# zerr0o/whisper-burn

Measured on AMD Instinct MI355X. Metric: real-time factor (audio-s/wall-s) Whisper Large-V3 Q4 @1/2/4/8 MI355X, higher is better.
Workload: dtype fp16x2

## Files before the change

### include/whisper_amd.h

```cpp
#ifndef WHISPER_AMD_H
#define WHISPER_AMD_H

#include <stddef.h>
#include <stdint.h>

#include "wq4.h"

#ifdef __cplusplus
extern "C" {
#endif

typedef struct wa_model wa_model;

typedef enum wa_variant { WA_LARGE_V3 = 0, WA_MEDIUM = 1, WA_TINY_TEST = 2 } wa_variant;

enum {
  WA_CFG_N_MELS = 0,
  WA_CFG_N_AUDIO_CTX,
  WA_CFG_N_AUDIO_STATE,
  WA_CFG_N_AUDIO_HEAD,
  WA_CFG_N_AUDIO_LAYER,
  WA_CFG_N_TEXT_CTX,
  WA_CFG_N_TEXT_STATE,
  WA_CFG_N_TEXT_HEAD,
  WA_CFG_N_TEXT_LAYER,
  WA_CFG_N_VOCAB,
  WA_CFG_N_LANG,
  WA_CFG_COUNT
};

const char* wa_last_error(void);

wq4_status wa_model_create_synthetic(int device, int variant, uint64_t seed, int max_batch, wq4_precision prec,
                                     wa_model** out);
wq4_status wa_model_create_synthetic_ex(int device, int variant, uint64_t seed, int max_batch, wq4_precision prec,
                                        int weight_type, wa_model** out);
int wa_model_weight_type(const wa_model* m);
int wa_model_wide_range(const wa_model* m);
wq4_status wa_model_create_from_gguf(int device, const char* path, int variant, int max_batch, wq4_precision prec,
                                     wa_model** out);
void wa_model_destroy(wa_model* m);

typedef struct wa_gguf wa_gguf;
wq4_status wa_gguf_open(const char* path, wa_gguf** out);
void wa_gguf_close(wa_gguf* g);
int wa_gguf_version(const wa_gguf* g);
int64_t wa_gguf_tensor_count(const wa_gguf* g);
wq4_status wa_gguf_tensor_info(const wa_gguf* g, int64_t index, char* name, size_t name_cap, int* ndims,
                               uint64_t* dims, int* type, uint64_t* offset, uint64_t* nbytes);
wq4_status wa_gguf_tensor_data(const wa_gguf* g, const char* name, uint8_t* out, size_t cap);
wq4_status wa_model_config(const wa_model* m, int32_t* cfg );
size_t wa_model_device_bytes(const wa_model* m);

wq4_status wa_transcribe(wa_model* m, const float* mel_dev, int n_clips, int lang_token, int max_tokens,
                         int eot_stop, int32_t* tokens_out, int32_t* n_tokens_out, void* stream);

wq4_status wa_transcribe_batches(wa_model* m, const float* mel_dev, int n_batches, int n_clips, int lang_token,
                                 int max_tokens, int eot_stop, int32_t* tokens_out, int32_t* n_tokens_out,
                                 void* stream);
wq4_status wa_last_pipeline_stats(const wa_model* m, float* out );
int wa_last_pipeline_pairs(const wa_model* m);

wq4_status wa_log_mel(int device, const float* audio_dev, int n_clips, int64_t n_samples, int64_t ld_audio,
                      int n_mels, float* mel_dev, void* stream);
wq4_status wa_mel_filterbank(int n_mels, float* filters_out, float* window_out);

wq4_status wa_last_timings(const wa_model* m, float* out );

#define WA_PROF_CATEGORIES 4
wq4_status wa_profile_enable(wa_model* m, int enable);
wq4_status wa_profile_read(wa_model* m, double* out , int reset);

#define WA_PROBE_OUT 6
wq4_status wa_probe_kernels(wa_model* m, int n_clips, int iters, double* out, int out_len);
int wa_decode_group_rows(int n_clips);

wq4_status wa_encode(wa_model* m, const float* mel_dev, int n_clips, float* enc_out_dev, void* stream);
wq4_status wa_prompt_logits(wa_model* m, const int32_t* prompt_dev, int n_clips, int plen, float* logits_dev,
                            void* stream);
wq4_status wa_xattn_check(int device, const float* q_dev, const uint8_t* wk_dev, const uint8_t* wv_dev,
                          const float* bv_dev, int weight_type, const float* enc_dev, int n_clips, int Tq, int T,
                          int H, wq4_precision prec, float* out_dev);
int wa_xattn_resident_share(int live_clips, int T, int planes, int D, double budget_mb);
int wa_xattn_chunk_resident(int chunk, int share);
wq4_status wa_xattn_plan(int T, int* splits, int* chunks_per_split);
wq4_status wa_xattn_plan_splits(int T, int rows, int free_cus, int* splits, int* chunks_per_split);
long long wa_decode_graph_key(const wa_model* m, int group);
wq4_status wa_xattn_kv_check(int device, const float* q_dev, const float* k_dev, const float* v_dev, int n_clips,
                             int Tq, int T, int H, wq4_precision prec, float* out_dev);

wq4_status wa_transcribe_trace(wa_model* m, const float* mel_dev, int n_clips, int lang_token, int max_tokens,
                               int eot_stop, int32_t* tokens_out, int32_t* n_tokens_out, const int32_t* trace_ids_dev,
                               int trace_k, float* trace_out_dev, void* stream);
wq4_status wa_encoder_attention_check(int device, const float* qkv_dev, int n_clips, int T, int H, wq4_precision prec,
                                      float* out_dev);
wq4_status wa_self_attention_check(int device, const float* qkv_dev, float* cache_k_dev, float* cache_v_dev,
                                   int n_clips, int Tq, int H, int ctx, int kv_len, wq4_precision prec,
                                   float* out_dev);
wq4_status wa_logits_argmax_check(int device, const float* hid_dev, const float* emb_dev, int n_clips, int D, int V,
                                  int step, wq4_precision prec, int32_t* tok_dev, float* logits_dev);
wq4_status wa_synth_uniform(uint64_t seed, const char* name, int64_t n, float lo, float hi, float* out);

#ifdef __cplusplus
}
#endif
#endif
```

### whisper-burn_amd/csrc/whisper/wa_api.cpp

```cpp
#include "wa_model.hpp"

using namespace wa;

namespace {

thread_local std::string g_err;

wq4_status create_model(int device, int variant, int max_batch, wq4_precision prec, int weight_type, Source& src,
                        wa_model** out) {
  WA_HIP(hipSetDevice(device));
  std::unique_ptr<wa_model> m(new wa_model());
  m->device = device;
  m->cfg = preset(variant);
  m->prec = prec;
  m->ns = prec == WQ4_PREC_F16 ? 1 : 2;
  m->bmax = max_batch;
  kv_config(m.get(), max_batch);
  m->wtype = weight_type;
  WA_TRY(build_model(m.get(), src));
  WA_TRY(build_ln_fold(m.get()));
  WA_TRY(alloc_activations(m.get()));
  WA_HIP(hipStreamCreateWithFlags(&m->own_stream, hipStreamNonBlocking));
  WA_HIP(hipDeviceSynchronize());
  *out = m.release();
  return WQ4_OK;
}

}

wq4_status wa::fail(wq4_status s, const std::string& m) {
  g_err = m;
  return s;
}

extern "C" {

const char* wa_last_error(void) { return g_err.c_str(); }

wq4_status wa_model_create_synthetic_ex(int device, int variant, uint64_t seed, int max_batch, wq4_precision prec,
                                        int weight_type, wa_model** out) {
  if (!out) return fail(WQ4_EINVAL, "out is null");
  *out = nullptr;
  if (variant < 0 || variant > 2) return fail(WQ4_EINVAL, "unknown variant");
  if (max_batch < 1 || max_batch > 256) return fail(WQ4_EINVAL, "max_batch must be in [1, 256]");
  if (prec != WQ4_PREC_F16X2 && prec != WQ4_PREC_F16) return fail(WQ4_EINVAL, "unknown precision");
  if (weight_type != 0 && weight_type != 1) return fail(WQ4_EINVAL, "weight_type must be 0 (Q4_0) or 1 (F16)");
  return create_model(device, variant, max_batch, prec, weight_type, *synth_source(seed), out);
}

wq4_status wa_model_create_synthetic(int device, int variant, uint64_t seed, int max_batch, wq4_precision prec,
                                     wa_model** out) {
  return wa_model_create_synthetic_ex(device, variant, seed, max_batch, prec, 0, out);
}

wq4_status wa_model_create_from_gguf(int device, const char* path, int variant, int max_batch, wq4_precision prec,
                                     wa_model** out) {
  if (!out || !path) return fail(WQ4_EINVAL, "null argument");
  *out = nullptr;
  if (variant < 0 || variant > 2) return fail(WQ4_EINVAL, "unknown variant");
  if (max_batch < 1 || max_batch > 256) return fail(WQ4_EINVAL, "max_batch must be in [1, 256]");
  if (prec != WQ4_PREC_F16X2 && prec != WQ4_PREC_F16) return fail(WQ4_EINVAL, "unknown precision");
  GgufFile file;
  if (!file.open(path)) return fail(WQ4_EINVAL, "Failed to parse GGUF: " + file.error());
  const GgufTensor* probe = file.find("encoder.blocks.0.attn.query.weight");
  const int wtype = probe && probe->type == kGgmlF16 ? 1 : 0;
  return create_model(device, variant, max_batch, prec, wtype, *gguf_source(file), out);
}

void wa_model_destroy(wa_model* m) { delete m; }

wq4_status wa_gguf_open(const char* path, wa_gguf** out) {
  if (!path || !out) return fail(WQ4_EINVAL, "null argument");
  *out = nullptr;
  auto* f = new GgufFile();
  if (!f->open(path)) {
    const std::string e = f->error();
    delete f;
    return fail(WQ4_EINVAL, "Failed to parse GGUF: " + e);
  }
  *out = reinterpret_cast<wa_gguf*>(f);
  return WQ4_OK;
}

void wa_gguf_close(wa_gguf* g) { delete reinterpret_cast<GgufFile*>(g); }

int wa_gguf_version(const wa_gguf* g) { return g ? (int)reinterpret_cast<const GgufFile*>(g)->version() : -1; }

int64_t wa_gguf_tensor_count(const wa_gguf* g) {
  return g ? (int64_t)reinterpret_cast<const GgufFile*>(g)->tensors().size() : -1;
}

wq4_status wa_gguf_tensor_info(const wa_gguf* g, int64_t index, char* name, size_t name_cap, int* ndims,
                               uint64_t* dims, int* type, uint64_t* offset, uint64_t* nbytes) {
  if (!g) return fail(WQ4_EINVAL, "null gguf");
  const auto& ts = reinterpret_cast<const GgufFile*>(g)->tensors();
  if (index < 0 || index >= (int64_t)ts.size()) return fail(WQ4_EINVAL, "tensor index out of range");
  const GgufTensor& t = ts[(size_t)index];
  if (name && name_cap) {
    const size_t n = std::min(name_cap - 1, t.name.size());
    std::memcpy(name, t.name.data(), n);
    name[n] = 0;
  }
  if (ndims) *ndims = (int)t.dims.size();
  if (dims)
    for (size_t i = 0; i < t.dims.size(); ++i) dims[i] = t.dims[i];
  if (type) *type = (int)t.type;
  if (offset) *offset = t.offset;
  if (nbytes) *nbytes = t.nbytes();
  return WQ4_OK;
}

wq4_status wa_gguf_tensor_data(const wa_gguf* g, const char* name, uint8_t* out, size_t cap) {
  if (!g || !name || !out) return fail(WQ4_EINVAL, "null argument");
  const auto* f = reinterpret_cast<const GgufFile*>(g);
  const GgufTensor* t = f->find(name);
  if (!t) return fail(WQ4_EINVAL, std::string("Tensor '") + name + "' not found in GGUF");
  const uint8_t* p = f->data(*t);
  if (!p) return fail(WQ4_EINVAL, std::string("Tensor '") + name + "' data lies outside the file");
  if (cap < t->nbytes()) return fail(WQ4_ENOMEM, "output buffer too small");
  std::memcpy(out, p, t->nbytes());
  return WQ4_OK;
}

int wa_model_weight_type(const wa_model* m) { return m ? m->wtype : -1; }

int wa_model_wide_range(const wa_model* m) { return m ? m->range_tier : -1; }

wq4_status wa_model_config(const wa_model* m, int32_t* cfg) {
  if (!m || !cfg) return fail(WQ4_EINVAL, "null argument");
  const Config& c = m->cfg;
  const int32_t v[WA_CFG_COUNT] = {c.n_mels,       c.n_audio_ctx,  c.n_audio_state, c.n_audio_head,
                                   c.n_audio_layer, c.n_text_ctx,   c.n_text_state,  c.n_text_head,
                                   c.n_text_layer,  c.n_vocab,      c.n_lang};
  std::memcpy(cfg, v, sizeof(v));
  return WQ4_OK;
}

size_t wa_model_device_bytes(const wa_model* m) { return m ? m->bytes : 0; }

wq4_status wa_last_timings(const wa_model* m, float* out) {
  if (!m || !out) return fail(WQ4_EINVAL, "null argument");
  std::memcpy(out, m->timings, sizeof(m->timings));
  return WQ4_OK;
}

wq4_status wa_profile_enable(wa_model* m, int enable) {
  if (!m) return fail(WQ4_EINVAL, "null model");
  m->profile = enable != 0;
  return WQ4_OK;
}

wq4_status wa_profile_read(wa_model* m, double* out, int reset) {
  if (!m || !out) return fail(WQ4_EINVAL, "null argument");
  m->resolve_profile();
  std::memcpy(out, m->prof, sizeof(m->prof));
  if (reset) std::memset(m->prof, 0, sizeof(m->prof));
  return WQ4_OK;
}

wq4_status wa_encode(wa_model* m, const float* mel_dev, int n_clips, float* enc_out_dev, void* stream) {
  if (!m || !mel_dev) return fail(WQ4_EINVAL, "null argument");
  if (n_clips < 1 || n_clips > m->bmax) return fail(WQ4_EINVAL, "n_clips out of range");
  WA_HIP(hipSetDevice(m->device));
  hipStream_t st = static_cast<hipStream_t>(stream);
  WA_TRY(encoder_forward(m, mel_dev, n_clips, st, enc_out_dev));
  return cross_kv_forward(m, n_clips, st, false);
}

wq4_status wa_prompt_logits(wa_model* m, const int32_t* prompt_dev, int n_clips, int plen, float* logits_dev,
                            void* stream) {
  if (!m || !prompt_dev || !logits_dev) return fail(WQ4_EINVAL, "null argument");
  if (n_clips < 1 || n_clips > m->bmax || plen < 1 || plen > 4) return fail(WQ4_EINVAL, "bad n_clips / plen");
  if (n_clips > m->kv_batch) return fail(WQ4_EINVAL, "wa_encode the clips first");
  WA_HIP(hipSetDevice(m->device));
  hipStream_t st = static_cast<hipStream_t>(stream);
  DecGroup& g = m->groups[0];
  g.lane = 0;
  g.b0 = 0;
  g.nb = n_clips;
  g.xres = xattn_residency(n_clips, m->cfg.n_audio_ctx, m->ns, m->cfg.n_audio_state);
  g.xplan = xattn_plan(m->cfg.n_audio_ctx, n_clips);
  WA_TRY(decoder_forward(m, g, prompt_dev, plen, nullptr, 0, 0, st));
  WA_HIP(hipMemcpyAsync(logits_dev, g.logits, (size_t)n_clips * m->cfg.n_vocab * 4, hipMemcpyDeviceToDevice, st));
  return WQ4_OK;
}

int wa_decode_group_rows(int n_clips) {
  if (n_clips < 1) return 0;
  const int G = decode_groups(n_clips);
  return (n_clips + G - 1) / G;
}

constexpr int kProbeOut = WA_PROBE_OUT;

wq4_status wa_probe_kernels(wa_model* m, int n_clips, int iters, double* out, int out_len) {
  if (!m || !out) return fail(WQ4_EINVAL, "null argument");
  if (out_len < kProbeOut) return fail(WQ4_EINVAL, "out holds fewer than 6 doubles");
  if (n_clips < 1 || n_clips > m->bmax || iters < 1) return fail(WQ4_EINVAL, "bad n_clips / iters");
  if (n_clips > m->kv_batch) return fail(WQ4_EINVAL, "run wa_transcribe / wa_encode on n_clips clips first");
  WA_HIP(hipSetDevice(m->device));
  hipStream_t st = m->own_stream;
  const Config& c = m->cfg;
  const int B = n_clips, D = c.n_text_state, T = c.n_audio_ctx, H = c.n_text_head;
  DecLayer& L = m->dec[0];
  DecGroup g = m->groups[0];
  const _Float16* enc = m->enc_planes;
  hipEvent_t a, b;
  WA_HIP(hipEventCreate(&a));
  WA_HIP(hipEventCreate(&b));
  float ms = 0.0f;
  g.b0 = 0;
  g.nb = B;
  const bool kv = m->group_kv(g);
  const XattnResidency res = xattn_residency(B, T, m->ns, D);
  const XattnPlan plan = xattn_plan(T, B);
  auto xattn = [&]() -> hipError_t {
    if (kv)
      return launch_cross_attention_kv(g.qd, L.xk, L.xv, B, 1, T, H, g.xkv_part, g.xkv_ctr, g.atd_dec, m->ns, st);
    return launch_xattn(g.qd, L.ck_raw, L.cv_raw, L.cv_p, L.cv_b, m->wtype, enc, B, 1, T, H, D, g.xqt, g.xattn_part,
                        g.atd_dec, m->ns, res, plan, st);
  };
  WA_HIP(xattn());
  WA_HIP(hipEventRecord(a, st));
  for (int i = 0; i < iters; ++i) WA_HIP(xattn());
  WA_HIP(hipEventRecord(b, st));
  WA_HIP(hipEventSynchronize(b));
  WA_HIP(hipEventElapsedTime(&ms, a, b));
  out[0] = ms * 1e3 / iters;
  const double wbytes = m->wtype == 1 ? 2.0 * D * D * 2 : 2.0 * D * D * 18 / 32;
  out[1] = kv ? (double)B * T * D * 4 * 2 + (double)B * D * (4 + 2 * m->ns)
              : (double)B * T * D * 2 * m->ns + wbytes + (double)B * D * (4 + 2 * m->ns);
  out[5] = kv ? 1.0 : 0.0;
  const int F = 4 * D;
  WA_WQ4(wq4_gemm_tiled(L.fc1, L.fc1_b, g.atd_dec, nullptr, nullptr, g.atf_dec, B, WQ4_EPI_GELU | WQ4_EPI_TILED_OUT,
                        m->prec, 2, st));
  WA_HIP(hipEventRecord(a, st));
  for (int i = 0; i < iters; ++i)
    WA_WQ4(wq4_gemm_tiled(L.fc1, L.fc1_b, g.atd_dec, nullptr, nullptr, g.atf_dec, B,
                          WQ4_EPI_GELU | WQ4_EPI_TILED_OUT, m->prec, 2, st));
  WA_HIP(hipEventRecord(b, st));
  WA_HIP(hipEventSynchronize(b));
  WA_HIP(hipEventElapsedTime(&ms, a, b));
  out[2] = ms * 1e3 / iters;
  out[3] = (double)F * D * 18 / 32 + (double)B * D * 2 * m->ns + (double)B * F * 2 * m->ns;
  out[4] = 2.0 * B * F * D;
  (void)hipEventDestroy(a);
  (void)hipEventDestroy(b);
  return WQ4_OK;
}

}
```

### whisper-burn_amd/csrc/whisper/wa_forward.cpp

```cpp
#include "wa_model.hpp"

using namespace wa;

namespace {

constexpr int kSOT = 50258;

struct Prof {
  wa_model* m;
  hipStream_t st;
  int cat;
  double gflop, gb;
  hipEvent_t a = nullptr, b = nullptr;
  Prof(wa_model* m_, hipStream_t st_, int cat_, double gflop_, double gb_)
      : m(m_), st(st_), cat(cat_), gflop(gflop_), gb(gb_) {
    if (m->profile && st != m->enc_stream && hipEventCreate(&a) == hipSuccess && hipEventCreate(&b) == hipSuccess)
      (void)hipEventRecord(a, st);
  }
  ~Prof() {
    if (a && b) {
      (void)hipEventRecord(b, st);
      m->pending.push_back({a, b, cat, gflop, gb});
    }
  }
};

Prof q4prof(wa_model* m, hipStream_t st, const wq4_tensor* w, int64_t rows) {
  int64_t n = 0, k = 0;
  (void)wq4_tensor_shape(w, &n, &k);
  return Prof(m, st, 0, 2.0 * rows * n * k * 1e-9, ((double)n * k * 18 / 32 + 4.0 * rows * k + 4.0 * rows * n) * 1e-9);
}

bool lnfold_on(const wa_model* m, int Tq, const DecodeState* state, int64_t rows) {
  static const bool enabled = [] {
    const char* e = getenv("WA_LN_FOLD");
    return e ? atoi(e) != 0 : true;
  }();
  if (!enabled || !m->fold_allowed() || state == nullptr || Tq != 1 || m->dec.empty()) return false;
  const DecLayer& L = m->dec[0];
  for (const wq4_tensor* w : {L.qkv, L.out, L.cq, L.cout, L.fc1, L.fc2})
    if (!wq4_lnfold_supported(w, rows)) return false;
  return true;
}

bool fused_pick(const DecGroup& g, int Tq, const DecodeState* state) {
  return state != nullptr && Tq == 1 && g.nb <= 32;
}

wq4_status decode_step(wa_model* m, DecGroup& g, int eot_stop, hipStream_t st) {
  WA_HIP(launch_bookkeep(g.next_tok, g.tokens, g.ntok, g.done, g.nb, kMaxTokens, eot_stop, g.state, st));
  WA_TRY(decoder_forward(m, g, g.next_tok, 1, g.state, 0, 0, st));
  if (!fused_pick(g, 1, g.state))
    WA_HIP(launch_argmax_step(g.logits, g.nb, m->cfg.n_vocab, kMinTokens, g.state, g.next_tok, m->range_flag, st));
  return WQ4_OK;
}

}

namespace wa {

wq4_status alloc_activations(wa_model* m) {
  const Config& c = m->cfg;
  const int D = c.n_audio_state, F = 4 * D, Dt = c.n_text_state, Ft = 4 * Dt;
  const int B = m->bmax, T = c.n_audio_ctx;
  const int64_t renc = (int64_t)B * T, rdec = (int64_t)B * 4;
  Dev& d = m->dev;
  auto tiled = [&](int64_t rows, int k) {
    const size_t n = wq4_atiled_bytes(rows, k, m->prec);
    m->bytes += n;
    return d.alloc<_Float16>(n / 2);
  };
  auto f32 = [&](int64_t n) {
    m->bytes += (size_t)n * 4;
    return d.alloc<float>((size_t)n);
  };
  m->h1 = f32((int64_t)B * 2 * T * D);
  m->x = f32(renc * D);
  m->qkv = f32(renc * 3 * D);
  m->at_d = tiled(renc, D);
  m->at_f = tiled(renc, F);
  m->enc_planes = d.alloc<_Float16>((size_t)renc * m->ns * D);
  m->bytes += (size_t)renc * m->ns * D * 2;
  for (auto& L : m->dec) {
    L.cache_k = f32((int64_t)B * c.n_text_ctx * Dt);
    L.cache_v = f32((int64_t)B * c.n_text_ctx * Dt);
  }
  if (!emb_tiled_supported(Dt)) return fail(WQ4_EINVAL, "n_text_state must be a multiple of 128");
  const size_t erows = (size_t)emb_tiled_rows(c.n_vocab);
  m->tok_emb2 = d.alloc<_Float16>(erows * m->ns * Dt);
  if (!m->tok_emb2) return fail(WQ4_ENOMEM, "embedding plane allocation failed");
  m->bytes += erows * m->ns * Dt * 2;
  WA_HIP(launch_emb_tiled(m->tok_emb, c.n_vocab, Dt, m->ns, m->tok_emb2, nullptr));
  const int HP = (c.n_text_head + 15) / 16 * 16;
  size_t xpart = 0;
  for (int r = 1; r <= rdec; ++r) xpart = std::max(xpart, xattn_part_floats(r, c.n_text_head, Dt, T));
  m->groups.resize(kMaxGroups);
  for (DecGroup& g : m->groups) {
    g.xd = f32(rdec * Dt);
    g.qkvd = f32(rdec * 3 * Dt);
    g.qd = f32(rdec * Dt);
    g.hid = f32(rdec * Dt);
    g.logits = f32((int64_t)B * c.n_vocab);
    g.atd_dec = tiled(rdec, Dt);
    g.atf_dec = tiled(rdec, Ft);
    g.prompt_tok = d.alloc<int>(rdec);
    g.next_tok = d.alloc<int>(B);
    g.tokens = d.alloc<int>((size_t)B * kMaxTokens);
    g.ntok = d.alloc<int>(B);
    g.done = d.alloc<int>(B);
    g.state = d.alloc<DecodeState>(1);
    g.xattn_part = f32((int64_t)xpart);
    const int kvc = std::max(1, m->kv_clips);
    g.xkv_part = f32((int64_t)cross_attention_kv_part_floats(kvc, c.n_text_head, T));
    g.xkv_ctr = d.alloc<int>((size_t)kvc * c.n_text_head);
    g.xqt = d.alloc<_Float16>((size_t)rdec * m->ns * HP * Dt);
    g.atd_ln = tiled(rdec, Dt);
    g.ln_stats = f32(rdec * (Dt / 16) * 2);
    g.hid_t = tiled(rdec, Dt);
    g.lg_val = f32((int64_t)32 * logits_argmax_groups(c.n_vocab));
    g.lg_idx = d.alloc<int>((size_t)32 * logits_argmax_groups(c.n_vocab));
    g.lg_ctr = d.alloc<int>(1);
    m->bytes += (size_t)rdec * m->ns * HP * Dt * 2;
    for (void* p : {(void*)g.xd, (void*)g.qkvd, (void*)g.qd, (void*)g.hid, (void*)g.logits, (void*)g.atd_dec,
                    (void*)g.atf_dec, (void*)g.prompt_tok, (void*)g.next_tok, (void*)g.tokens, (void*)g.ntok,
                    (void*)g.done, (void*)g.state, (void*)g.xattn_part, (void*)g.xqt, (void*)g.lg_val,
                    (void*)g.lg_idx, (void*)g.lg_ctr, (void*)g.atd_ln, (void*)g.ln_stats, (void*)g.hid_t,
                    (void*)g.xkv_part, (void*)g.xkv_ctr})
      if (!p) return fail(WQ4_ENOMEM, "decode-group allocation failed");
    WA_HIP(hipMemset(g.xkv_ctr, 0, (size_t)kvc * c.n_text_head * sizeof(int)));
    WA_HIP(hipMemset(g.atd_ln, 0, wq4_atiled_bytes(rdec, Dt, m->prec)));
    WA_HIP(hipMemset(g.hid_t, 0, wq4_atiled_bytes(rdec, Dt, m->prec)));
    WA_HIP(hipMemset(g.lg_ctr, 0, sizeof(int)));
    WA_HIP(hipMemset(g.xqt, 0, (size_t)rdec * m->ns * HP * Dt * 2));
    WA_HIP(hipMemset(g.atd_dec, 0, wq4_atiled_bytes(rdec, Dt, m->prec)));
    WA_HIP(hipMemset(g.atf_dec, 0, wq4_atiled_bytes(rdec, Ft, m->prec)));
    WA_HIP(hipHostMalloc(reinterpret_cast<void**>(&g.host_ndone), 8 * sizeof(int), 0));
    WA_HIP(hipStreamCreateWithFlags(&g.st, hipStreamNonBlocking));
  }
  m->range_flag = d.alloc<int>(1);
  for (void* p : {(void*)m->h1, (void*)m->x, (void*)m->qkv, (void*)m->at_d, (void*)m->at_f, (void*)m->enc_planes,
                  (void*)m->range_flag})
    if (!p) return fail(WQ4_ENOMEM, "activation allocation failed");
  WA_HIP(hipMemset(m->range_flag, 0, sizeof(int)));
  for (auto& L : m->dec)
    if (!L.cache_k || !L.cache_v) return fail(WQ4_ENOMEM, "KV cache allocation failed");
  WA_HIP(hipMemset(m->at_d, 0, wq4_atiled_bytes(renc, D, m->prec)));
  WA_HIP(hipMemset(m->at_f, 0, wq4_atiled_bytes(renc, F, m->prec)));
  return WQ4_OK;
}

wq4_status encoder_front(wa_model* m, const float* mel, int B, hipStream_t st) {
  const Config& c = m->cfg;
  const int D = c.n_audio_state, T = c.n_audio_ctx;
  const int T_mel = 2 * T;
  const int64_t rows = (int64_t)B * T;
  {
    Prof p(m, st, 2, 2.0 * B * T_mel * D * 3.0 * c.n_mels * 1e-9, 4.0 * B * T_mel * (c.n_mels + D) * 1e-9);
    WA_HIP(launch_conv_gelu(mel, (long)c.n_mels * T_mel, T_mel, 1, B, c.n_mels, T_mel, 1, m->conv1_wt, m->conv1_b,
                            nullptr, D, m->h1, st));
  }
  {
    Prof p(m, st, 2, 2.0 * rows * D * 3.0 * D * 1e-9, 4.0 * B * (T_mel + T) * D * 1e-9);
    WA_HIP(launch_conv_gelu(m->h1, (long)T_mel * D, 1, D, B, D, T_mel, 2, m->conv2_wt, m->conv2_b, m->enc_pos, D,
                            m->x, st));
  }
  return WQ4_OK;
}

wq4_status encoder_layers(wa_model* m, int B, int l0, int l1, hipStream_t st) {
  const Config& c = m->cfg;
  const int D = c.n_audio_state, T = c.n_audio_ctx, H = c.n_audio_head;
  const int64_t rows = (int64_t)B * T;
  const double ln_gb = 8.0 * rows * D * 1e-9;
  for (int li = l0; li < l1; ++li) {
    const EncLayer& L = m->enc[li];
    {
      Prof p(m, st, 3, 0.0, ln_gb);
      WA_WQ4(wq4_layernorm(m->x, L.ln1_w, L.ln1_b, rows, D, m->prec, m->at_d, nullptr, st));
    }
    {
      Prof p = q4prof(m, st, L.qkv, rows);
      WA_WQ4(wq4_gemm_tiled(L.qkv, L.qkv_b, m->at_d, nullptr, m->qkv, nullptr, rows, 0u, m->prec, 1, st));
    }
    {
      Prof p(m, st, 1, 4.0 * B * H * (double)T * T * 64 * 1e-9, 16.0 * rows * D * 1e-9);
      WA_HIP(launch_encoder_attention(m->qkv, B, T, H, m->at_d, m->ns, st, m->f32_attn() ? m->h1 : nullptr));
    }
    if (m->f32_attn()) {
      WA_WQ4(wq4_linear_forward_ws(L.out, L.out_b, m->h1, m->x, m->x, rows, D, WQ4_EPI_RESIDUAL, m->prec, m->at_d,
                                   wq4_atiled_bytes(rows, D, m->prec), st));
    } else {
      Prof p = q4prof(m, st, L.out, rows);
      WA_WQ4(wq4_gemm_tiled(L.out, L.out_b, m->at_d, m->x, m->x, nullptr, rows, WQ4_EPI_RESIDUAL, m->prec, 1, st));
    }
    if (m->abi_ffn()) {
      WA_WQ4(wq4_layernorm(m->x, L.ln2_w, L.ln2_b, rows, D, WQ4_PREC_F16X2, nullptr, m->qkv, st));
      WA_WQ4(wq4_ffn_forward_ws(L.fc1, L.fc1_b, L.fc2, L.fc2_b, m->qkv, m->x, m->x, rows, WQ4_EPI_RESIDUAL, m->prec,
                                m->ffn_ws, m->ffn_ws_bytes, st));
      continue;
    }
    {
      Prof p(m, st, 3, 0.0, ln_gb);
      WA_WQ4(wq4_layernorm(m->x, L.ln2_w, L.ln2_b, rows, D, m->prec, m->at_d, nullptr, st));
    }
    {
      Prof p = q4prof(m, st, L.fc1, rows);
      WA_WQ4(wq4_gemm_tiled(L.fc1, L.fc1_b, m->at_d, nullptr, nullptr, m->at_f, rows,
                            WQ4_EPI_GELU | WQ4_EPI_TILED_OUT, m->prec, 1, st));
    }
    {
      Prof p = q4prof(m, st, L.fc2, rows);
      WA_WQ4(wq4_gemm_tiled(L.fc2, L.fc2_b, m->at_f, m->x, m->x, nullptr, rows, WQ4_EPI_RESIDUAL, m->prec, 1, st));
    }
  }
  return WQ4_OK;
}

wq4_status encoder_post(wa_model* m, int B, hipStream_t st, float* enc_out_f32) {
  const Config& c = m->cfg;
  const int D = c.n_audio_state;
  const int64_t rows = (int64_t)B * c.n_audio_ctx;
  Prof p(m, st, 3, 0.0, 8.0 * rows * D * 1e-9);
  float* out = enc_out_f32 ? enc_out_f32 : m->h1;
  WA_WQ4(wq4_layernorm(m->x, m->lnp_w, m->lnp_b, rows, D, WQ4_PREC_F16X2, nullptr, out, st));
  m->enc_f32 = out;
  return WQ4_OK;
}

wq4_status encoder_forward(wa_model* m, const float* mel, int B, hipStream_t st, float* enc_out_f32) {
  WA_TRY(encoder_front(m, mel, B, st));
  WA_TRY(encoder_layers(m, B, 0, (int)m->enc.size(), st));
  return encoder_post(m, B, st, enc_out_f32);
}

wq4_status cross_kv_forward(wa_model* m, int B, hipStream_t st, bool caches, int lane) {
  const Config& c = m->cfg;
  const int64_t rows = (int64_t)B * c.n_audio_ctx;
  if (lane == 1) {
    WA_HIP(launch_enc_planes(m->enc_f32, rows, c.n_audio_state, m->ns, m->enc_planes2, st));
    return WQ4_OK;
  }
  m->kv_batch = B;
  WA_HIP(launch_enc_planes(m->enc_f32, rows, c.n_audio_state, m->ns, m->enc_planes, st));
  m->kv_n = caches && B <= m->kv_small ? B : 0;
  if (m->kv_n > 0 && !m->kv_alloc_ok) {
    const size_t n = (size_t)m->kv_clips * c.n_audio_ctx * c.n_text_state;
    bool ok = true;
    for (DecLayer& L : m->dec) {
      if (!L.xk) L.xk = m->dev.alloc<float>(n);
      if (!L.xv) L.xv = m->dev.alloc<float>(n);
      if (!L.xk || !L.xv) {
        ok = false;
        break;
      }
    }
    if (!ok) {
      for (DecLayer& L : m->dec) {
        m->dev.release(L.xk);
        m->dev.release(L.xv);
        L.xk = L.xv = nullptr;
      }
      m->kv_n = 0;
      return fail(WQ4_ENOMEM, "cross K/V cache allocation failed");
    }
    m->bytes += n * 8 * m->dec.size();
    m->kv_alloc_ok = true;
  }
  if (m->kv_n > 0) {
    const int64_t kv_rows = (int64_t)m->kv_n * c.n_audio_ctx;
    WA_WQ4(wq4_layernorm(m->x, m->lnp_w, m->lnp_b, kv_rows, c.n_audio_state, m->prec, m->at_d, nullptr, st));
    for (DecLayer& L : m->dec) {
      WA_WQ4(wq4_gemm_tiled_headmajor(L.ck, nullptr, m->at_d, L.xk, kv_rows, c.n_audio_ctx, c.n_text_state, m->prec,
                                      0, st));
      WA_WQ4(wq4_gemm_tiled_headmajor(L.cv, L.cv_b, m->at_d, L.xv, kv_rows, c.n_audio_ctx, c.n_text_state, m->prec,
                                      0, st));
    }
  }
  return WQ4_OK;
}

wq4_status decoder_forward(wa_model* m, DecGroup& g, const int* tokens, int Tq, const DecodeState* state, int pos0,
                           int kv0, hipStream_t st) {
  const Config& c = m->cfg;
  const int D = c.n_text_state, H = c.n_text_head, T = c.n_audio_ctx;
  const int B = g.nb;
  const int64_t rows = (int64_t)B * Tq;
  const size_t self_ofs = (size_t)g.b0 * H * c.n_text_ctx * 64;
  const _Float16* enc = (g.lane ? m->enc_planes2 : m->enc_planes) + (size_t)g.b0 * T * m->ns * c.n_audio_state;
  const bool fold = lnfold_on(m, Tq, state, rows);
  float* const a32 = m->f32_attn() ? g.hid : nullptr;
  auto ln_gemm = [&](const wq4_tensor* w, const float* bias, const float* wg, const float* b2, const float* lw,
                     const float* lb, float* y, void* yt, unsigned flags) -> wq4_status {
    if (fold) {
      const wq4_ln_fold cons{nullptr, nullptr, nullptr, g.ln_stats, wg};
      WA_WQ4(wq4_gemm_tiled_lnfold(w, b2, g.atd_ln, nullptr, y, yt, rows, flags, m->prec, &cons, st));
    } else {
      WA_WQ4(wq4_layernorm(g.xd, lw, lb, rows, D, m->prec, g.atd_dec, nullptr, st));
      WA_WQ4(wq4_gemm_tiled(w, bias, g.atd_dec, nullptr, y, yt, rows, flags, m->prec, 2, st));
    }
    return WQ4_OK;
  };
  auto resid_gemm = [&](const wq4_tensor* w, const float* bias, const void* at, const float* x32,
                        const float* next_lw) -> wq4_status {
    if (x32) {
      WA_WQ4(wq4_linear_forward_ws(w, bias, x32, g.xd, g.xd, rows, D, WQ4_EPI_RESIDUAL, m->prec, g.atd_dec,
                                   wq4_atiled_bytes(rows, D, m->prec), st));
    } else if (fold) {
      const wq4_ln_fold prod{next_lw, next_lw ? g.atd_ln : nullptr, next_lw ? g.ln_stats : nullptr, nullptr, nullptr};
      WA_WQ4(wq4_gemm_tiled_lnfold(w, bias, at, g.xd, g.xd, nullptr, rows, WQ4_EPI_RESIDUAL, m->prec, &prod, st));
    } else {
      WA_WQ4(wq4_gemm_tiled(w, bias, at, g.xd, g.xd, nullptr, rows, WQ4_EPI_RESIDUAL, m->prec, 2, st));
    }
    return WQ4_OK;
  };
  if (fold)
    WA_HIP(launch_embed_fold(tokens, m->tok_emb, m->dec_pos, B, Tq, D, state, pos0, g.xd, m->dec[0].ln1_w, g.atd_ln,
                             g.ln_stats, m->ns, st));
  else
    WA_HIP(launch_embed(tokens, m->tok_emb, m->dec_pos, B, Tq, D, state, pos0, g.xd, st));
  const int nl = (int)m->dec.size();
  for (int li = 0; li < nl; ++li) {
    DecLayer& L = m->dec[li];
    WA_TRY(ln_gemm(L.qkv, L.qkv_b, L.qkv_wg, L.qkv_b2, L.ln1_w, L.ln1_b, g.qkvd, nullptr, 0u));
    WA_HIP(launch_decoder_self_attention(g.qkvd, (g.lane ? L.cache_k2 : L.cache_k) + self_ofs,
                                         (g.lane ? L.cache_v2 : L.cache_v) + self_ofs, B, Tq, H, c.n_text_ctx, state,
                                         kv0, g.atd_dec, m->ns, st, a32));
    WA_TRY(resid_gemm(L.out, L.out_b, g.atd_dec, a32, L.ln2_w));
    WA_TRY(ln_gemm(L.cq, L.cq_b, L.cq_wg, L.cq_b2, L.ln2_w, L.ln2_b, g.qd, nullptr, 0u));
    if (m->group_kv(g)) {
      const size_t kofs = (size_t)g.b0 * T * D;
      WA_HIP(launch_cross_attention_kv(g.qd, L.xk + kofs, L.xv + kofs, B, Tq, T, H, g.xkv_part, g.xkv_ctr, g.atd_dec,
                                       m->ns, st, a32));
    } else {
      WA_HIP(launch_xattn(g.qd, L.ck_raw, L.cv_raw, L.cv_p, L.cv_b, m->wtype, enc, B, Tq, T, H, D, g.xqt,
                          g.xattn_part, g.atd_dec, m->ns, g.xres, g.xplan, st, a32));
    }
    WA_TRY(resid_gemm(L.cout, L.cout_b, g.atd_dec, a32, L.ln3_w));
    if (m->abi_ffn()) {
      WA_WQ4(wq4_layernorm(g.xd, L.ln3_w, L.ln3_b, rows, D, WQ4_PREC_F16X2, nullptr, g.hid, st));
      WA_WQ4(wq4_ffn_forward_ws(L.fc1, L.fc1_b, L.fc2, L.fc2_b, g.hid, g.xd, g.xd, rows, WQ4_EPI_RESIDUAL, m->prec,
                                g.ffn_ws, g.ffn_ws_bytes, st));
      continue;
    }
    WA_TRY(ln_gemm(L.fc1, L.fc1_b, L.fc1_wg, L.fc1_b2, L.ln3_w, L.ln3_b, nullptr, g.atf_dec,
                   WQ4_EPI_GELU | WQ4_EPI_TILED_OUT));
    WA_TRY(resid_gemm(L.fc2, L.fc2_b, g.atf_dec, nullptr, li + 1 < nl ? m->dec[li + 1].ln1_w : nullptr));
  }
  if (fused_pick(g, Tq, state)) {
    WA_WQ4(wq4_layernorm(g.xd, m->dln_w, m->dln_b, rows, D, m->prec, g.hid_t, nullptr, st));
    const size_t tofs = (size_t)g.b0 * m->trace_s1 * m->trace_k;
    WA_HIP(launch_logits_argmax(g.hid_t, B, D, m->tok_emb2, m->ns, c.n_vocab, kMinTokens, state, g.lg_val, g.lg_idx,
                                g.lg_ctr, g.next_tok, m->trace_out ? m->trace_ids + tofs : nullptr,
                                m->trace_out ? m->trace_out + tofs : nullptr, m->trace_s1, m->trace_k, m->range_flag,
                                st));
    return WQ4_OK;
  }
  WA_WQ4(wq4_layernorm(g.xd, m->dln_w, m->dln_b, rows, D, WQ4_PREC_F16X2, nullptr, g.hid, st));
  WA_HIP(launch_logits(g.hid + (size_t)(Tq - 1) * D, B, D, (int64_t)Tq * D, m->tok_emb, c.n_vocab, g.logits, st));
  return WQ4_OK;
}

wq4_status prompt_group(wa_model* m, DecGroup& g, int lang_token, hipStream_t st) {
  const Config& c = m->cfg;
  const int B = g.nb;
  std::vector<int> ptok((size_t)B * 4);
  int pos0, kv0;
  if (lang_token >= 0) {
    for (int b = 0; b < B; ++b) {
      ptok[b * 4 + 0] = kSOT;
      ptok[b * 4 + 1] = lang_token;
      ptok[b * 4 + 2] = c.transcribe_token();
      ptok[b * 4 + 3] = c.no_timestamps_token();
    }
    WA_HIP(hipMemcpyAsync(g.prompt_tok, ptok.data(), (size_t)B * 4 * 4, hipMemcpyHostToDevice, st));
    WA_TRY(decoder_forward(m, g, g.prompt_tok, 4, nullptr, 0, 0, st));
    pos0 = 4;
    kv0 = 4;
  } else {
    for (int b = 0; b < B; ++b) {
      ptok[b * 3 + 0] = kSOT;
      ptok[b * 3 + 1] = c.transcribe_token();
      ptok[b * 3 + 2] = c.no_timestamps_token();
    }
    WA_HIP(hipMemcpyAsync(g.prompt_tok, ptok.data(), (size_t)B * 3 * 4, hipMemcpyHostToDevice, st));
    std::vector<int> sot(B, kSOT);
    WA_HIP(hipMemcpyAsync(g.next_tok, sot.data(), (size_t)B * 4, hipMemcpyHostToDevice, st));
    WA_TRY(decoder_forward(m, g, g.next_tok, 1, nullptr, 0, 0, st));
    WA_HIP(launch_argmax(g.logits, B, c.n_vocab, 50259, 50259 + c.n_lang, 0, nullptr, g.prompt_tok, 3, m->range_flag,
                         st));
    WA_TRY(decoder_forward(m, g, g.prompt_tok, 3, nullptr, 0, 0, st));
    pos0 = 4;
    kv0 = 3;
  }
  WA_HIP(launch_argmax(g.logits, B, c.n_vocab, 0, c.n_vocab, 1, nullptr, g.next_tok, 1, m->range_flag, st));
  const DecodeState init{pos0 - 1, kv0 - 1, -1, 0};
  WA_HIP(hipMemcpyAsync(g.state, &init, sizeof(init), hipMemcpyHostToDevice, st));
  WA_HIP(hipMemsetAsync(g.ntok, 0, (size_t)B * 4, st));
  WA_HIP(hipMemsetAsync(g.done, 0, (size_t)B * 4, st));
  WA_HIP(hipMemsetAsync(g.tokens, 0, (size_t)B * kMaxTokens * 4, st));
  return WQ4_OK;
}

wq4_status ensure_graph(wa_model* m, DecGroup& g, int eot_stop) {
  const int64_t key =
      ((((((((int64_t)g.lane * 512 + g.b0) * 512 + g.nb) * 2 + (eot_stop ? 1 : 0)) * 2 + (m->trace_out ? 1 : 0)) * 2 +
         (m->group_kv(g) ? 1 : 0)) * 4 + m->range_tier) * 16 + g.xplan.splits) * (kXattnResDen + 1) + g.xres.q;
  if (g.graph && g.graph_key == key) return WQ4_OK;
  std::swap(g.graph, g.graph_alt);
  std::swap(g.graph_key, g.graph_alt_key);
  if (g.graph && g.graph_key == key) return WQ4_OK;
  if (g.graph) {
    (void)hipGraphExecDestroy(g.graph);
    g.graph = nullptr;
  }
  WA_WQ4(wq4_prepare_stream(m->device, g.st));
  hipGraph_t gr;
  WA_HIP(hipStreamBeginCapture(g.st, hipStreamCaptureModeThreadLocal));
  wq4_status s = decode_step(m, g, eot_stop, g.st);
  hipError_t ce = hipStreamEndCapture(g.st, &gr);
  if (s != WQ4_OK) return s;
  if (ce != hipSuccess) return fail(WQ4_EHIP, std::string("graph capture: ") + hipGetErrorString(ce));
  ce = hipGraphInstantiate(&g.graph, gr, nullptr, nullptr, 0);
  (void)hipGraphDestroy(gr);
  if (ce != hipSuccess) return fail(WQ4_EHIP, std::string("graph instantiate: ") + hipGetErrorString(ce));
  g.graph_key = key;
  return WQ4_OK;
}

void kv_config(wa_model* m, int max_batch) {
  static const int small = [] {
    const char* e = getenv("WA_XATTN_KV_CLIPS");
    return e ? std::max(0, atoi(e)) : 8;
  }();
  m->kv_small = std::min(small, max_batch);
  m->kv_clips = m->kv_small;
}

wq4_status ensure_ffn_ws(wa_model* m) {
  if (m->ffn_ws) return WQ4_OK;
  const DecLayer& Ld = m->dec.front();
  const EncLayer& Le = m->enc.front();
  const size_t ne = wq4_ffn_workspace_bytes(Le.fc1, Le.fc2, (int64_t)m->bmax * m->cfg.n_audio_ctx);
  const size_t nd = wq4_ffn_workspace_bytes(Ld.fc1, Ld.fc2, (int64_t)m->bmax * 4);
  if (ne == 0 || nd == 0) return fail(WQ4_EINVAL, "FFN workspace size");
  void* e = m->dev.alloc<uint8_t>(ne);
  bool ok = e != nullptr;
  for (DecGroup& g : m->groups) {
    g.ffn_ws = ok ? m->dev.alloc<uint8_t>(nd) : nullptr;
    ok = ok && g.ffn_ws != nullptr;
  }
  if (!ok) {
    m->dev.release(e);
    for (DecGroup& g : m->groups) {
      m->dev.release(g.ffn_ws);
      g.ffn_ws = nullptr;
      g.ffn_ws_bytes = 0;
    }
    return fail(WQ4_ENOMEM, "range tier 2: FFN workspace allocation failed");
  }
  for (DecGroup& g : m->groups) {
    g.ffn_ws_bytes = nd;
    m->bytes += nd;
  }
  m->ffn_ws = e;
  m->ffn_ws_bytes = ne;
  m->bytes += ne;
  return WQ4_OK;
}

bool ensure_pair_lane(wa_model* m) {
  if (m->enc_planes2) return true;
  const Config& c = m->cfg;
  const size_t np = (size_t)m->bmax * c.n_audio_ctx * m->ns * c.n_audio_state;
  const size_t nc = (size_t)m->bmax * c.n_text_ctx * c.n_text_state;
  _Float16* planes = m->dev.alloc<_Float16>(np);
  bool ok = planes != nullptr;
  for (DecLayer& L : m->dec) {
    if (!ok) break;
    L.cache_k2 = m->dev.alloc<float>(nc);
    L.cache_v2 = m->dev.alloc<float>(nc);
    ok = L.cache_k2 && L.cache_v2;
  }
  if (!ok) {
    (void)hipGetLastError();
    m->dev.release(planes);
    for (DecLayer& L : m->dec) {
      m->dev.release(L.cache_k2);
      m->dev.release(L.cache_v2);
      L.cache_k2 = L.cache_v2 = nullptr;
    }
    return false;
  }
  m->enc_planes2 = planes;
  m->bytes += np * 2 + nc * 8 * m->dec.size();
  return true;
}

int decode_groups(int B) {
  static const int forced = [] {
    const char* env = getenv("WA_DECODE_GROUPS");
    return env ? atoi(env) : 0;
  }();
  int G = forced > 0 ? forced : (B >= 16 ? 2 : 1);
  if (G > kMaxGroups) G = kMaxGroups;
  if (G > B) G = B;
  return G;
}

}
```

### whisper-burn_amd/csrc/whisper/wa_model.hpp

```cpp
#pragma once
#include <hip/hip_runtime_api.h>

#include <algorithm>
#include <cstring>
#include <memory>
#include <string>
#include <vector>

#include "../../../include/whisper_amd.h"
#include "../../../include/wq4.h"
#include "wa_gguf.hpp"
#include "wa_kernels.hpp"

namespace wa {

wq4_status fail(wq4_status s, const std::string& m);

#define WA_HIP(expr)                                                                                \
  do {                                                                                              \
    hipError_t e_ = (expr);                                                                         \
    if (e_ != hipSuccess) return wa::fail(WQ4_EHIP, std::string(#expr) + ": " + hipGetErrorString(e_)); \
  } while (0)
#define WA_WQ4(expr)                                                                    \
  do {                                                                                  \
    wq4_status s_ = (expr);                                                             \
    if (s_ != WQ4_OK) return wa::fail(s_, std::string(#expr) + ": " + wq4_last_error()); \
  } while (0)
#define WA_TRY(expr)             \
  do {                           \
    wq4_status s_ = (expr);      \
    if (s_ != WQ4_OK) return s_; \
  } while (0)

constexpr int kMaxTokens = 224;
constexpr int kMinTokens = 3;

struct Config {
  int n_mels, n_audio_ctx, n_audio_state, n_audio_head, n_audio_layer;
  int n_text_ctx, n_text_state, n_text_head, n_text_layer, n_vocab, n_lang;
  int transcribe_token() const { return 50260 + n_lang; }
  int no_timestamps_token() const { return transcribe_token() + 4; }
};

struct Dev {
  std::vector<void*> ptrs;
  ~Dev() {
    for (void* p : ptrs) (void)hipFree(p);
  }
  template <class T>
  T* alloc(size_t n) {
    void* p = nullptr;
    if (hipMalloc(&p, n * sizeof(T) + 256) != hipSuccess) return nullptr;
    ptrs.push_back(p);
    return static_cast<T*>(p);
  }
  void release(void* p) {
    if (!p) return;
    for (void*& q : ptrs)
      if (q == p) {
        (void)hipFree(q);
        q = ptrs.back();
        ptrs.pop_back();
        return;
      }
  }
};

struct EncLayer {
  float *ln1_w, *ln1_b, *ln2_w, *ln2_b, *qkv_b, *out_b, *fc1_b, *fc2_b;
  wq4_tensor *qkv = nullptr, *out = nullptr, *fc1 = nullptr, *fc2 = nullptr;
};
struct DecLayer {
  float *ln1_w, *ln1_b, *ln2_w, *ln2_b, *ln3_w, *ln3_b;
  float *qkv_b, *out_b, *cq_b, *cv_b, *cout_b, *fc1_b, *fc2_b;
  wq4_tensor *qkv = nullptr, *out = nullptr, *cq = nullptr, *cout = nullptr, *fc1 = nullptr, *fc2 = nullptr;
  float *qkv_wg = nullptr, *qkv_b2 = nullptr, *cq_wg = nullptr, *cq_b2 = nullptr, *fc1_wg = nullptr,
        *fc1_b2 = nullptr;
  uint8_t *ck_raw = nullptr, *cv_raw = nullptr;
  uint32_t* cv_p = nullptr;
  float *cache_k, *cache_v;
  float *cache_k2 = nullptr, *cache_v2 = nullptr;
  wq4_tensor *ck = nullptr, *cv = nullptr;
  float *xk = nullptr, *xv = nullptr;
};

constexpr int kMaxGroups = 4;
struct DecGroup {
  hipStream_t st = nullptr;
  int b0 = 0, nb = 0;
  int lane = 0;
  XattnResidency xres;
  XattnPlan xplan{0, 0};
  float *xd, *qkvd, *qd, *hid, *logits;
  _Float16 *atd_dec, *atf_dec;
  int *prompt_tok, *next_tok, *tokens, *ntok, *done;
  _Float16* xqt;
  float* xattn_part;
  float* xkv_part;
  int* xkv_ctr;
  _Float16* atd_ln;
  float* ln_stats;
  _Float16* hid_t;
  float* lg_val;
  int *lg_idx, *lg_ctr;
  DecodeState* state;
  void* ffn_ws = nullptr;
  size_t ffn_ws_bytes = 0;
  int* host_ndone = nullptr;
  hipGraphExec_t graph = nullptr;
  int64_t graph_key = -1;
  hipGraphExec_t graph_alt = nullptr;
  int64_t graph_alt_key = -1;
};

}

struct wa_model {
  int device = 0;
  wa::Config cfg{};
  wq4_precision prec = WQ4_PREC_F16X2;
  int ns = 2;
  int bmax = 1;
  wa::Dev dev;
  size_t bytes = 0;
  float *conv1_wt, *conv1_b, *conv2_wt, *conv2_b, *enc_pos, *lnp_w, *lnp_b;
  float *tok_emb, *dec_pos, *dln_w, *dln_b;
  _Float16* tok_emb2 = nullptr;
  std::vector<wa::EncLayer> enc;
  std::vector<wa::DecLayer> dec;
  float *h1, *x, *qkv;
  _Float16 *at_d, *at_f;
  _Float16* enc_planes = nullptr;
  _Float16* enc_planes2 = nullptr;
  const float* enc_f32 = nullptr;
  std::vector<wa::DecGroup> groups;
  int wtype = 0;
  int kv_batch = 0;
  int kv_clips = 0, kv_small = 0;
  int kv_n = 0;
  bool kv_alloc_ok = false;
  bool group_kv(const wa::DecGroup& g) const { return g.nb > 0 && g.b0 + g.nb <= kv_n; }
  hipStream_t own_stream = nullptr;
  hipStream_t enc_stream = nullptr;
  int enc_cus = 0;
  int dev_cus = 0;
  int overlap_k = -1;
  int overlap_b = 0, overlap_eot = -1;
  float pipe[4] = {0, 0, 0, 0};
  int pipe_pairs = 0;
  int* range_flag = nullptr;
  int range_tier = 0;
  bool fold_allowed() const { return range_tier < 1; }
  bool abi_ffn() const { return range_tier >= 2; }
  bool f32_attn() const { return range_tier >= 3; }
  void* ffn_ws = nullptr;
  size_t ffn_ws_bytes = 0;
  float timings[5] = {0, 0, 0, 0, 0};
  const int* trace_ids = nullptr;
  float* trace_out = nullptr;
  int trace_s1 = 0, trace_k = 0;
  struct Pending {
    hipEvent_t a, b;
    int cat;
    double gflop, gb;
  };
  bool profile = false;
  std::vector<Pending> pending;
  double prof[WA_PROF_CATEGORIES][4] = {};

  void resolve_profile() {
    for (auto& p : pending) {
      float ms = 0.0f;
      if (hipEventSynchronize(p.b) == hipSuccess && hipEventElapsedTime(&ms, p.a, p.b) == hipSuccess) {
        prof[p.cat][0] += 1;
        prof[p.cat][1] += ms;
        prof[p.cat][2] += p.gflop;
        prof[p.cat][3] += p.gb;
      }
      (void)hipEventDestroy(p.a);
      (void)hipEventDestroy(p.b);
    }
    pending.clear();
  }

  ~wa_model() {
    resolve_profile();
    for (auto& g : groups) {
      if (g.graph) (void)hipGraphExecDestroy(g.graph);
      if (g.graph_alt) (void)hipGraphExecDestroy(g.graph_alt);
      if (g.st) (void)hipStreamDestroy(g.st);
      if (g.host_ndone) (void)hipHostFree(g.host_ndone);
    }
    if (own_stream) (void)hipStreamDestroy(own_stream);
    if (enc_stream) (void)hipStreamDestroy(enc_stream);
    for (auto& l : enc)
      for (wq4_tensor* t : {l.qkv, l.out, l.fc1, l.fc2}) wq4_tensor_destroy(t);
    for (auto& l : dec)
      for (wq4_tensor* t : {l.qkv, l.out, l.cq, l.cout, l.fc1, l.fc2, l.ck, l.cv}) wq4_tensor_destroy(t);
  }
};

namespace wa {

Config preset(int variant);
struct Source {
  virtual ~Source() = default;
  virtual bool f32(const std::string& name, int64_t n, float lo, float hi, bool optional, std::vector<float>& out) = 0;
  virtual bool linear(const std::string& name, int rows, int k, int wtype, uint8_t* dst) = 0;
  std::string err;
};
std::unique_ptr<Source> synth_source(uint64_t seed);
std::unique_ptr<Source> gguf_source(const GgufFile& f);
wq4_status build_model(wa_model* m, Source& src);
wq4_status build_ln_fold(wa_model* m);

void kv_config(wa_model* m, int max_batch);
wq4_status alloc_activations(wa_model* m);
wq4_status ensure_ffn_ws(wa_model* m);
int decode_groups(int B);
wq4_status encoder_front(wa_model* m, const float* mel, int B, hipStream_t st);
wq4_status encoder_layers(wa_model* m, int B, int l0, int l1, hipStream_t st);
wq4_status encoder_post(wa_model* m, int B, hipStream_t st, float* enc_out_f32);
wq4_status encoder_forward(wa_model* m, const float* mel, int B, hipStream_t st, float* enc_out_f32);
wq4_status cross_kv_forward(wa_model* m, int B, hipStream_t st, bool caches, int lane = 0);
bool ensure_pair_lane(wa_model* m);
wq4_status decoder_forward(wa_model* m, DecGroup& g, const int* tokens, int Tq, const DecodeState* state, int pos0,
                           int kv0, hipStream_t st);
wq4_status prompt_group(wa_model* m, DecGroup& g, int lang_token, hipStream_t st);
wq4_status ensure_graph(wa_model* m, DecGroup& g, int eot_stop);

}
```

### whisper-burn_amd/csrc/whisper/wa_transcribe.cpp

```cpp
#include "wa_model.hpp"

using namespace wa;

namespace {

constexpr int kEncOverlapCUs = 32;
constexpr int kEncOverlapLayers0 = 16;
constexpr double kEncOverlapFill = 0.98;
constexpr int kXattnPeerCUs = 64;

struct EventSet {
  std::vector<hipEvent_t> e;
  EventSet() = default;
  EventSet(const EventSet&) = delete;
  EventSet& operator=(const EventSet&) = delete;
  ~EventSet() {
    for (hipEvent_t x : e) (void)hipEventDestroy(x);
  }
  hipError_t make(hipEvent_t* out, bool timing = true) {
    hipError_t r = hipEventCreateWithFlags(out, timing ? hipEventDefault : hipEventDisableTiming);
    if (r == hipSuccess) e.push_back(*out);
    return r;
  }
};

constexpr int kPairMinClips = 16, kPairMaxClips = 32;

bool pair_enabled() {
  static const bool enabled = [] {
    const char* e = getenv("WA_PAIR_BATCHES");
    return e ? atoi(e) != 0 : true;
  }();
  return enabled;
}

int unit_groups(int B, bool pair) { return pair ? 2 : decode_groups(B); }

wq4_status run_decode(wa_model* m, int B, bool pair, int masked_cus, int lang_token, int max_tokens, int eot_stop,
                      hipEvent_t ready, const hipEvent_t* gprompt, const hipEvent_t* gdone, int* gsteps) {
  const int G = unit_groups(B, pair);
  const XattnResidency xres = xattn_residency(pair ? 2 * B : B, m->cfg.n_audio_ctx, m->ns, m->cfg.n_audio_state);
  if (m->dev_cus <= 0) WA_HIP(hipDeviceGetAttribute(&m->dev_cus, hipDeviceAttributeMultiprocessorCount, m->device));
  const int rows = pair ? B : (B + G - 1) / G;
  const int free_cus = std::max(1, m->dev_cus - masked_cus - (G > 1 ? kXattnPeerCUs : 0));
  const XattnPlan xplan = xattn_plan(m->cfg.n_audio_ctx, rows, free_cus);
  for (int i = 0; i < G; ++i) {
    DecGroup& g = m->groups[i];
    g.xres = xres;
    g.xplan = xplan;
    g.lane = pair ? i : 0;
    g.b0 = pair ? 0 : (int)((int64_t)B * i / G);
    g.nb = pair ? B : (int)((int64_t)B * (i + 1) / G) - g.b0;
    WA_HIP(hipStreamWaitEvent(g.st, ready, 0));
    WA_TRY(prompt_group(m, g, lang_token, g.st));
    WA_HIP(hipEventRecord(gprompt[i], g.st));
    WA_TRY(ensure_graph(m, g, eot_stop));
  }
  EventSet ev;
  hipEvent_t ring[kMaxGroups][8];
  if (eot_stop)
    for (int i = 0; i < G; ++i)
      for (auto& e : ring[i]) WA_HIP(ev.make(&e, false));
  const int lag = 4;
  bool live[kMaxGroups] = {};
  int nlive = G;
  for (int i = 0; i < G; ++i) {
    live[i] = true;
    gsteps[i] = 0;
  }
  for (int step = 0; step < max_tokens && nlive > 0; ++step) {
    for (int i = 0; i < G; ++i) {
      if (!live[i]) continue;
      DecGroup& g = m->groups[i];
      WA_HIP(hipGraphLaunch(g.graph, g.st));
      ++gsteps[i];
      if (eot_stop) {
        const int slot = step % 8;
        WA_HIP(hipMemcpyAsync(&g.host_ndone[slot], &g.state->n_done, sizeof(int), hipMemcpyDeviceToHost, g.st));
        WA_HIP(hipEventRecord(ring[i][slot], g.st));
      }
    }
    if (eot_stop && step >= lag) {
      const int old = (step - lag) % 8;
      for (int i = 0; i < G; ++i) {
        if (!live[i]) continue;
        WA_HIP(hipEventSynchronize(ring[i][old]));
        if (m->groups[i].host_ndone[old] >= m->groups[i].nb) {
          live[i] = false;
          --nlive;
        }
      }
    }
  }
  for (int i = 0; i < G; ++i) WA_HIP(hipEventRecord(gdone[i], m->groups[i].st));
  return WQ4_OK;
}

wq4_status collect_batch(wa_model* m, int B, bool pair, const hipEvent_t* gdone, hipStream_t st, int32_t* tok,
                         int32_t* nt, int* flag, size_t lane_stride) {
  const int G = unit_groups(B, pair);
  for (int i = 0; i < G; ++i) WA_HIP(hipStreamWaitEvent(st, gdone[i], 0));
  for (int i = 0; i < G; ++i) {
    const DecGroup& g = m->groups[i];
    const size_t ofs = g.lane * lane_stride;
    WA_HIP(hipMemcpyAsync(tok + ofs + (size_t)g.b0 * kMaxTokens, g.tokens, (size_t)g.nb * kMaxTokens * 4,
                          hipMemcpyDeviceToHost, st));
    WA_HIP(hipMemcpyAsync(nt + ofs + g.b0, g.ntok, (size_t)g.nb * 4, hipMemcpyDeviceToHost, st));
  }
  for (int i = 0; i < (pair ? 2 : 1); ++i)
    WA_HIP(hipMemcpyAsync(flag + i * lane_stride, m->range_flag, sizeof(int), hipMemcpyDeviceToHost, st));
  return WQ4_OK;
}

void copy_tokens(const int32_t* tok, const int32_t* nt, int B, int max_tokens, int32_t* tokens_out,
                 int32_t* n_tokens_out) {
  for (int b = 0; b < B; ++b) {
    n_tokens_out[b] = std::min(nt[b], max_tokens);
    std::memcpy(tokens_out + (size_t)b * max_tokens, tok + (size_t)b * kMaxTokens, (size_t)max_tokens * 4);
  }
}

wq4_status transcribe_once(wa_model* m, const float* mel_dev, int n_clips, int lang_token, int max_tokens,
                           int eot_stop, int32_t* tokens_out, int32_t* n_tokens_out, void* stream, bool* overflow) {
  hipStream_t st = m->own_stream;
  const int B = n_clips;
  const int G = decode_groups(B);
  EventSet ev;
  hipEvent_t e_in, e_enc, e_kv, e_ready, e_end, gprompt[kMaxGroups], gdone[kMaxGroups];
  for (hipEvent_t* e : {&e_in, &e_enc, &e_kv, &e_ready, &e_end}) WA_HIP(ev.make(e));
  for (int i = 0; i < G; ++i) {
    WA_HIP(ev.make(&gprompt[i]));
    WA_HIP(ev.make(&gdone[i]));
  }
  WA_HIP(hipEventRecord(e_in, static_cast<hipStream_t>(stream)));
  WA_HIP(hipStreamWaitEvent(st, e_in, 0));
  WA_HIP(hipMemsetAsync(m->range_flag, 0, sizeof(int), st));

  WA_HIP(hipEventRecord(e_enc, st));
  WA_TRY(encoder_forward(m, mel_dev, B, st, nullptr));
  WA_HIP(hipEventRecord(e_kv, st));
  WA_TRY(cross_kv_forward(m, B, st, true));
  WA_HIP(hipEventRecord(e_ready, st));
  int gsteps[kMaxGroups] = {};
  WA_TRY(run_decode(m, B, false, 0, lang_token, max_tokens, eot_stop, e_ready, gprompt, gdone, gsteps));
  const int steps = *std::max_element(gsteps, gsteps + G);
  std::vector<int32_t> tok((size_t)B * kMaxTokens), nt(B);
  int flag = 0;
  WA_TRY(collect_batch(m, B, false, gdone, st, tok.data(), nt.data(), &flag, 0));
  WA_HIP(hipEventRecord(e_end, st));
  WA_HIP(hipStreamSynchronize(st));
  *overflow = flag != 0;
  copy_tokens(tok.data(), nt.data(), B, max_tokens, tokens_out, n_tokens_out);
  float t_enc = 0.0f, t_kv = 0.0f, tp = 0.0f, tall = 0.0f;
  WA_HIP(hipEventElapsedTime(&t_enc, e_enc, e_kv));
  WA_HIP(hipEventElapsedTime(&t_kv, e_kv, e_ready));
  for (int i = 0; i < G; ++i) {
    float t = 0.0f;
    WA_HIP(hipEventElapsedTime(&t, e_ready, gprompt[i]));
    tp = std::max(tp, t);
  }
  WA_HIP(hipEventElapsedTime(&tall, e_ready, e_end));
  m->timings[0] = t_enc;
  m->timings[1] = t_kv;
  m->timings[2] = tp;
  m->timings[3] = tall - tp;
  m->timings[4] = (float)steps;
  return WQ4_OK;
}

wq4_status ensure_enc_stream(wa_model* m) {
  if (m->enc_stream) return WQ4_OK;
  hipDeviceProp_t prop;
  WA_HIP(hipGetDeviceProperties(&prop, m->device));
  const int total = prop.multiProcessorCount;
  int n = kEncOverlapCUs;
  if (const char* e = getenv("WA_ENC_CUS")) n = atoi(e);
  n = std::max(8, std::min(total, n));
  std::vector<uint32_t> mask((total + 31) / 32, 0u);
  for (int i = 0; i < n; ++i) mask[i / 32] |= 1u << (i % 32);
  WA_HIP(hipExtStreamCreateWithCUMask(&m->enc_stream, (uint32_t)mask.size(), mask.data()));
  m->enc_cus = n;
  return WQ4_OK;
}

wq4_status transcribe_pipelined(wa_model* m, const float* mel_dev, int NB, int B, int lang_token, int max_tokens,
                                int eot_stop, int32_t* tokens_out, int32_t* n_tokens_out, void* stream, int* flags) {
  WA_TRY(ensure_enc_stream(m));
  hipStream_t st = m->own_stream, es = m->enc_stream;
  const int L = (int)m->enc.size();
  const size_t mel_stride = (size_t)B * m->cfg.n_mels * 2 * m->cfg.n_audio_ctx;
  const bool pairing = pair_enabled() && NB >= 2 && B >= kPairMinClips && B <= kPairMaxClips && B > m->kv_small &&
                       decode_groups(B) == 2 && ensure_pair_lane(m);
  int32_t* host = nullptr;
  const size_t per = (size_t)B * kMaxTokens + B + 1;
  WA_HIP(hipHostMalloc(reinterpret_cast<void**>(&host), (size_t)NB * per * 4, 0));
  struct HostGuard {
    wa_model* m;
    int32_t* p;
    bool done = false;
    ~HostGuard() {
      if (!done) {
        (void)hipStreamSynchronize(m->own_stream);
        if (m->enc_stream) (void)hipStreamSynchronize(m->enc_stream);
        for (DecGroup& g : m->groups)
          if (g.st) (void)hipStreamSynchronize(g.st);
      }
      (void)hipHostFree(p);
    }
  } hg{m, host};
  EventSet ev;
  struct Unit {
    int first = 0, n = 1;
    hipEvent_t ready, mstart, mend, pstart, gprompt[kMaxGroups], gdone[kMaxGroups];
    int k = 0, gsteps[kMaxGroups] = {};
  };
  std::vector<Unit> ut;
  for (int i = 0; i < NB; i += ut.back().n) {
    ut.emplace_back();
    ut.back().first = i;
    ut.back().n = pairing && NB - i >= 2 ? 2 : 1;
  }
  const int NU = (int)ut.size();
  for (Unit& u : ut) {
    for (hipEvent_t* e : {&u.ready, &u.mstart, &u.mend, &u.pstart}) WA_HIP(ev.make(e));
    for (int i = 0; i < unit_groups(B, u.n == 2); ++i) {
      WA_HIP(ev.make(&u.gprompt[i]));
      WA_HIP(ev.make(&u.gdone[i]));
    }
  }
  auto unit_encoder = [&](Unit& u, int k0) -> wq4_status {
    for (int j = 0; j < u.n; ++j) {
      if (j == 0 && k0 >= 0) {
        WA_TRY(encoder_layers(m, B, k0, L, st));
        WA_TRY(encoder_post(m, B, st, nullptr));
      } else {
        WA_TRY(encoder_forward(m, mel_dev + (u.first + j) * mel_stride, B, st, nullptr));
      }
      WA_TRY(cross_kv_forward(m, B, st, true, j));
    }
    WA_HIP(hipMemsetAsync(m->range_flag, 0, sizeof(int), st));
    WA_HIP(hipEventRecord(u.ready, st));
    return WQ4_OK;
  };
  hipEvent_t e_in, e_enc0;
  WA_HIP(ev.make(&e_in));
  WA_HIP(ev.make(&e_enc0));
  WA_HIP(hipEventRecord(e_in, static_cast<hipStream_t>(stream)));
  WA_HIP(hipStreamWaitEvent(st, e_in, 0));
  WA_HIP(hipEventRecord(e_enc0, st));
  WA_TRY(unit_encoder(ut[0], -1));
  if (m->overlap_k < 0 || m->overlap_b != B || m->overlap_eot != eot_stop) m->overlap_k = std::min(L, kEncOverlapLayers0);
  m->overlap_b = B;
  m->overlap_eot = eot_stop;
  double t_exposed = 0.0, t_masked = 0.0, t_decode = 0.0, t_prompt = 0.0, k_sum = 0.0;
  int32_t steps_all = 0;
  for (int i = 0; i < NU; ++i) {
    Unit& u = ut[i];
    const bool pair = u.n == 2;
    if (i >= 1) {
      Unit& p = ut[i - 1];
      const int PG = unit_groups(B, p.n == 2);
      for (int g = 0; g < PG; ++g) WA_HIP(hipEventSynchronize(p.gdone[g]));
      WA_HIP(hipEventSynchronize(p.mend));
      float td = 0.0f, tm = 0.0f;
      for (int g = 0; g < PG; ++g) {
        float t = 0.0f;
        WA_HIP(hipEventElapsedTime(&t, p.ready, p.gdone[g]));
        td = std::max(td, t);
      }
      WA_HIP(hipEventElapsedTime(&tm, p.mstart, p.mend));
      if (!getenv("WA_ENC_OVERLAP")) {
        const double per_layer = tm / (double)(p.k + 1);
        double fill = kEncOverlapFill;
        if (const char* e = getenv("WA_ENC_FILL")) fill = atof(e);
        m->overlap_k = std::max(0, std::min(L, (int)(fill * td / per_layer) - 1));
      }
    }
    if (const char* e = getenv("WA_ENC_OVERLAP")) m->overlap_k = std::max(0, std::min(L, atoi(e)));
    if (i + 1 < NU) {
      u.k = m->overlap_k;
      WA_HIP(hipStreamWaitEvent(es, u.ready, 0));
      WA_HIP(hipEventRecord(u.mstart, es));
      WA_TRY(encoder_front(m, mel_dev + ut[i + 1].first * mel_stride, B, es));
      WA_TRY(encoder_layers(m, B, 0, u.k, es));
      WA_HIP(hipEventRecord(u.mend, es));
    }
    WA_TRY(run_decode(m, B, pair, i + 1 < NU ? m->enc_cus : 0, lang_token, max_tokens, eot_stop, u.ready, u.gprompt,
                      u.gdone, u.gsteps));
    int32_t* hb = host + (size_t)u.first * per;
    WA_TRY(collect_batch(m, B, pair, u.gdone, st, hb, hb + (size_t)B * kMaxTokens, hb + (size_t)B * kMaxTokens + B,
                         per));
    if (i + 1 < NU) {
      WA_HIP(hipStreamWaitEvent(st, u.mend, 0));
      WA_HIP(hipEventRecord(u.pstart, st));
      WA_TRY(unit_encoder(ut[i + 1], u.k));
    }
  }
  WA_HIP(hipStreamSynchronize(st));
  hg.done = true;
  for (int i = 0; i < NB; ++i) {
    const int32_t* hb = host + (size_t)i * per;
    copy_tokens(hb, hb + (size_t)B * kMaxTokens, B, max_tokens, tokens_out + (size_t)i * B * max_tokens,
                n_tokens_out + (size_t)i * B);
    flags[i] = hb[(size_t)B * kMaxTokens + B];
  }
  for (int i = 0; i < NU; ++i) {
    Unit& u = ut[i];
    const int UG = unit_groups(B, u.n == 2);
    float t = 0.0f, tp = 0.0f, td = 0.0f;
    if (i == 0) {
      WA_HIP(hipEventElapsedTime(&t, e_enc0, u.ready));
    } else {
      WA_HIP(hipEventElapsedTime(&t, ut[i - 1].pstart, u.ready));
      float tm = 0.0f;
      WA_HIP(hipEventElapsedTime(&tm, ut[i - 1].mstart, ut[i - 1].mend));
      t_masked += tm;
      k_sum += ut[i - 1].k;
    }
    t_exposed += t;
    for (int g = 0; g < UG; ++g) {
      float a = 0.0f, d = 0.0f;
      WA_HIP(hipEventElapsedTime(&a, u.ready, u.gprompt[g]));
      WA_HIP(hipEventElapsedTime(&d, u.ready, u.gdone[g]));
      tp = std::max(tp, a);
      td = std::max(td, d);
    }
    t_prompt += tp;
    t_decode += td - tp;
    steps_all += u.n == 2 ? u.gsteps[0] + u.gsteps[1] : *std::max_element(u.gsteps, u.gsteps + UG);
  }
  m->timings[0] = (float)(t_exposed / NB);
  m->timings[1] = 0.0f;
  m->timings[2] = (float)(t_prompt / NB);
  m->timings[3] = (float)(t_decode / NB);
  m->timings[4] = (float)steps_all / NB;
  m->pipe[0] = (float)NB;
  m->pipe[1] = NU > 1 ? (float)(k_sum / (NU - 1)) : 0.0f;
  m->pipe[2] = NU > 1 ? (float)(t_masked / (NU - 1)) : 0.0f;
  m->pipe[3] = (float)m->enc_cus;
  m->pipe_pairs = pairing ? NB / 2 : 0;
  return WQ4_OK;
}

}

extern "C" {

wq4_status wa_transcribe(wa_model* m, const float* mel_dev, int n_clips, int lang_token, int max_tokens,
                         int eot_stop, int32_t* tokens_out, int32_t* n_tokens_out, void* stream) {
  if (!m || !mel_dev || !tokens_out || !n_tokens_out) return fail(WQ4_EINVAL, "null argument");
  if (n_clips < 1 || n_clips > m->bmax) return fail(WQ4_EINVAL, "n_clips out of range");
  if (max_tokens < 1 || max_tokens > kMaxTokens) return fail(WQ4_EINVAL, "max_tokens must be in [1, 224]");
  WA_HIP(hipSetDevice(m->device));
  for (;;) {
    bool overflow = false;
    WA_TRY(transcribe_once(m, mel_dev, n_clips, lang_token, max_tokens, eot_stop, tokens_out, n_tokens_out, stream,
                           &overflow));
    if (!overflow) return WQ4_OK;
    if (m->range_tier == 3)
      return fail(WQ4_ERANGE,
                  "activation overflow: an MFMA operand left the f16-pair range (|x| >= 4094 after every range tier: "
                  "LayerNorm path, per-call FFN and attention-projection operand scales) and the logits are not finite");
    if (m->range_tier == 1) WA_TRY(ensure_ffn_ws(m));
    ++m->range_tier;
  }
}

wq4_status wa_transcribe_batches(wa_model* m, const float* mel_dev, int n_batches, int n_clips, int lang_token,
                                 int max_tokens, int eot_stop, int32_t* tokens_out, int32_t* n_tokens_out,
                                 void* stream) {
  if (!m || !mel_dev || !tokens_out || !n_tokens_out) return fail(WQ4_EINVAL, "null argument");
  if (n_batches < 1) return fail(WQ4_EINVAL, "n_batches must be >= 1");
  if (n_clips < 1 || n_clips > m->bmax) return fail(WQ4_EINVAL, "n_clips out of range");
  if (max_tokens < 1 || max_tokens > kMaxTokens) return fail(WQ4_EINVAL, "max_tokens must be in [1, 224]");
  WA_HIP(hipSetDevice(m->device));
  std::vector<int> flags(n_batches, 0);
  WA_TRY(transcribe_pipelined(m, mel_dev, n_batches, n_clips, lang_token, max_tokens, eot_stop, tokens_out,
                              n_tokens_out, stream, flags.data()));
  const size_t mel_stride = (size_t)n_clips * m->cfg.n_mels * 2 * m->cfg.n_audio_ctx;
  const int tier0 = m->range_tier;
  for (int i = 0; i < n_batches; ++i) {
    if (!flags[i] && m->range_tier == tier0) continue;
    WA_TRY(wa_transcribe(m, mel_dev + i * mel_stride, n_clips, lang_token, max_tokens, eot_stop,
                         tokens_out + (size_t)i * n_clips * max_tokens, n_tokens_out + (size_t)i * n_clips, stream));
  }
  return WQ4_OK;
}

wq4_status wa_last_pipeline_stats(const wa_model* m, float* out) {
  if (!m || !out) return fail(WQ4_EINVAL, "null argument");
  std::memcpy(out, m->pipe, sizeof(m->pipe));
  return WQ4_OK;
}

int wa_last_pipeline_pairs(const wa_model* m) { return m ? m->pipe_pairs : 0; }

wq4_status wa_transcribe_trace(wa_model* m, const float* mel_dev, int n_clips, int lang_token, int max_tokens,
                               int eot_stop, int32_t* tokens_out, int32_t* n_tokens_out, const int32_t* trace_ids_dev,
                               int trace_k, float* trace_out_dev, void* stream) {
  if (!m || !trace_ids_dev || !trace_out_dev || trace_k < 1) return fail(WQ4_EINVAL, "bad trace arguments");
  m->trace_ids = trace_ids_dev;
  m->trace_out = trace_out_dev;
  m->trace_s1 = max_tokens + 1;
  m->trace_k = trace_k;
  const wq4_status s = wa_transcribe(m, mel_dev, n_clips, lang_token, max_tokens, eot_stop, tokens_out,
                                     n_tokens_out, stream);
  m->trace_ids = nullptr;
  m->trace_out = nullptr;
  m->trace_s1 = m->trace_k = 0;
  for (DecGroup& g : m->groups) {
    for (hipGraphExec_t* x : {&g.graph, &g.graph_alt}) {
      if (*x) (void)hipGraphExecDestroy(*x);
      *x = nullptr;
    }
    g.graph_key = g.graph_alt_key = -1;
  }
  return s;
}

}
```

### whisper-burn_amd/whisper_amd/__init__.py

```python
from __future__ import annotations

import ctypes
import os
from typing import Optional

import numpy as np

import wq4

LIB_PATH = os.path.join(os.path.dirname(wq4.LIB_PATH), "libwhisper_amd.so")
HEADER_PATH = os.path.join(os.path.dirname(wq4.HEADER_PATH), "whisper_amd.h")
VARIANTS = {"large_v3": 0, "medium": 1, "tiny_test": 2}
CFG_KEYS = ["n_mels", "n_audio_ctx", "n_audio_state", "n_audio_head", "n_audio_layer", "n_text_ctx",
            "n_text_state", "n_text_head", "n_text_layer", "n_vocab", "n_lang"]
_lib: Optional[ctypes.CDLL] = None


def lib() -> ctypes.CDLL:
    global _lib
    if _lib is None:
        wq4.lib()
        if not os.path.exists(LIB_PATH):
            raise wq4.WQ4Error(6, f"{LIB_PATH} not built")
        L = ctypes.CDLL(LIB_PATH, mode=ctypes.RTLD_GLOBAL)
        vp, c_int, c_i64 = ctypes.c_void_p, ctypes.c_int, ctypes.c_int64
        i32p = ctypes.POINTER(ctypes.c_int32)
        f32p = ctypes.POINTER(ctypes.c_float)
        L.wa_last_error.restype = ctypes.c_char_p
        L.wa_model_create_synthetic.argtypes = [c_int, c_int, ctypes.c_uint64, c_int, c_int, ctypes.POINTER(vp)]
        L.wa_model_destroy.argtypes = [vp]
        L.wa_model_destroy.restype = None
        L.wa_model_config.argtypes = [vp, i32p]
        L.wa_model_device_bytes.argtypes = [vp]
        L.wa_model_device_bytes.restype = ctypes.c_size_t
        L.wa_transcribe.argtypes = [vp, vp, c_int, c_int, c_int, c_int, i32p, i32p, vp]
        L.wa_last_timings.argtypes = [vp, f32p]
        L.wa_transcribe_batches.argtypes = [vp, vp, c_int, c_int, c_int, c_int, c_int, i32p, i32p, vp]
        L.wa_last_pipeline_stats.argtypes = [vp, f32p]
        L.wa_last_pipeline_pairs.argtypes = [vp]
        L.wa_last_pipeline_pairs.restype = c_int
        L.wa_encode.argtypes = [vp, vp, c_int, vp, vp]
        L.wa_prompt_logits.argtypes = [vp, vp, c_int, c_int, vp, vp]
        L.wa_synth_uniform.argtypes = [ctypes.c_uint64, ctypes.c_char_p, c_i64, ctypes.c_float, ctypes.c_float, f32p]
        L.wa_profile_enable.argtypes = [vp, c_int]
        L.wa_profile_read.argtypes = [vp, ctypes.POINTER(ctypes.c_double), c_int]
        L.wa_probe_kernels.argtypes = [vp, c_int, c_int, ctypes.POINTER(ctypes.c_double), c_int]
        L.wa_decode_group_rows.argtypes = [c_int]
        L.wa_decode_group_rows.restype = c_int
        L.wa_model_create_synthetic_ex.argtypes = [c_int, c_int, ctypes.c_uint64, c_int, c_int, c_int,
                                                   ctypes.POINTER(vp)]
        L.wa_model_weight_type.argtypes = [vp]
        L.wa_model_weight_type.restype = c_int
        L.wa_model_wide_range.argtypes = [vp]
        L.wa_model_wide_range.restype = c_int
        L.wa_model_create_from_gguf.argtypes = [c_int, ctypes.c_char_p, c_int, c_int, c_int, ctypes.POINTER(vp)]
        L.wa_gguf_open.argtypes = [ctypes.c_char_p, ctypes.POINTER(vp)]
        L.wa_gguf_close.argtypes = [vp]
        L.wa_gguf_close.restype = None
        L.wa_gguf_version.argtypes = [vp]
        L.wa_gguf_version.restype = c_int
        L.wa_gguf_tensor_count.argtypes = [vp]
        L.wa_gguf_tensor_count.restype = c_i64
        L.wa_gguf_tensor_info.argtypes = [vp, c_i64, ctypes.c_char_p, ctypes.c_size_t, ctypes.POINTER(c_int),
                                          ctypes.POINTER(ctypes.c_uint64), ctypes.POINTER(c_int),
                                          ctypes.POINTER(ctypes.c_uint64), ctypes.POINTER(ctypes.c_uint64)]
        L.wa_gguf_tensor_data.argtypes = [vp, ctypes.c_char_p, ctypes.POINTER(ctypes.c_uint8), ctypes.c_size_t]
        L.wa_log_mel.argtypes = [c_int, vp, c_int, c_i64, c_i64, c_int, vp, vp]
        L.wa_mel_filterbank.argtypes = [c_int, f32p, f32p]
        L.wa_xattn_check.argtypes = [c_int, vp, vp, vp, vp, c_int, vp, c_int, c_int, c_int, c_int, c_int, vp]
        L.wa_xattn_resident_share.argtypes = [c_int, c_int, c_int, c_int, ctypes.c_double]
        L.wa_xattn_resident_share.restype = c_int
        L.wa_xattn_chunk_resident.argtypes = [c_int, c_int]
        L.wa_xattn_chunk_resident.restype = c_int
        L.wa_xattn_plan.argtypes = [c_int, ctypes.POINTER(c_int), ctypes.POINTER(c_int)]
        L.wa_xattn_plan.restype = c_int
        L.wa_xattn_plan_splits.argtypes = [c_int, c_int, c_int, ctypes.POINTER(c_int), ctypes.POINTER(c_int)]
        L.wa_xattn_plan_splits.restype = c_int
        L.wa_decode_graph_key.argtypes = [vp, c_int]
        L.wa_decode_graph_key.restype = ctypes.c_longlong
        L.wa_xattn_kv_check.argtypes = [c_int, vp, vp, vp, c_int, c_int, c_int, c_int, c_int, vp]
        L.wa_transcribe_trace.argtypes = [vp, vp, c_int, c_int, c_int, c_int, i32p, i32p, vp, c_int, vp, vp]
        L.wa_encoder_attention_check.argtypes = [c_int, vp, c_int, c_int, c_int, c_int, vp]
        L.wa_self_attention_check.argtypes = [c_int, vp, vp, vp, c_int, c_int, c_int, c_int, c_int, c_int, vp]
        L.wa_logits_argmax_check.argtypes = [c_int, vp, vp, c_int, c_int, c_int, c_int, c_int, vp, vp]
        for n in ("wa_xattn_check", "wa_xattn_kv_check", "wa_transcribe_trace", "wa_encoder_attention_check", "wa_self_attention_check",
                  "wa_logits_argmax_check", "wa_log_mel", "wa_mel_filterbank", "wa_model_create_synthetic", "wa_model_config", "wa_transcribe", "wa_transcribe_batches",
                  "wa_last_pipeline_stats", "wa_last_timings", "wa_encode",
                  "wa_prompt_logits", "wa_synth_uniform", "wa_profile_enable", "wa_profile_read", "wa_probe_kernels",
                  "wa_decode_group_rows",
                  "wa_model_create_from_gguf", "wa_model_create_synthetic_ex", "wa_gguf_open", "wa_gguf_tensor_info", "wa_gguf_tensor_data"):
            getattr(L, n).restype = c_int
        _lib = L
    return _lib


def check(st: int) -> None:
    if st != 0:
        raise wq4.WQ4Error(st, lib().wa_last_error().decode(errors="replace"))


def decode_group_rows(n_clips: int) -> int:
    return int(lib().wa_decode_group_rows(n_clips))


def synth_uniform(seed: int, name: str, n: int, lo: float, hi: float) -> np.ndarray:
    out = np.empty(n, np.float32)
    check(lib().wa_synth_uniform(seed, name.encode(), n, lo, hi, out.ctypes.data_as(ctypes.POINTER(ctypes.c_float))))
    return out


def _torch():
    import torch

    return torch


MEL_FRAMES = 3000
MEL_CHUNK = 480000


def mel_filterbank(n_mels: int = 128) -> tuple[np.ndarray, np.ndarray]:
    fb = np.empty((n_mels, 201), np.float32)
    win = np.empty(400, np.float32)
    f32p = ctypes.POINTER(ctypes.c_float)
    check(lib().wa_mel_filterbank(n_mels, fb.ctypes.data_as(f32p), win.ctypes.data_as(f32p)))
    return fb, win


def log_mel(audio, n_mels: int = 128, n_samples: Optional[int] = None, out=None):
    torch = _torch()
    assert audio.dtype == torch.float32 and audio.is_cuda and audio.dim() == 2
    if audio.stride(1) != 1:
        audio = audio.contiguous()
    B, L = audio.shape
    n = L if n_samples is None else int(n_samples)
    if out is None:
        out = torch.empty((B, n_mels, MEL_FRAMES), device=audio.device, dtype=torch.float32)
    dev = audio.device.index if audio.device.index is not None else torch.cuda.current_device()
    check(lib().wa_log_mel(dev, ctypes.c_void_p(audio.data_ptr()), B, n, audio.stride(0), n_mels,
                           ctypes.c_void_p(out.data_ptr()),
                           ctypes.c_void_p(torch.cuda.current_stream(audio.device).cuda_stream)))
    return out


def xattn_check(q, wk_raw, wv_raw, bv, enc, Tq: int, H: int, weight_type: int = 0,
                precision: int = wq4.PREC_F16X2):
    torch = _torch()
    B, T, D = enc.shape
    out = torch.empty((B * Tq, D), device=enc.device, dtype=torch.float32)
    dev = enc.device.index if enc.device.index is not None else 0
    ptr = lambda t: ctypes.c_void_p(t.contiguous().data_ptr())
    check(lib().wa_xattn_check(dev, ptr(q), ptr(wk_raw), ptr(wv_raw), ptr(bv), weight_type, ptr(enc), B, Tq, T, H,
                               precision, ptr(out)))
    return out


XATTN_SHARE_DEN = 64


def xattn_resident_share(live_clips: int, T: int, planes: int, D: int, budget_mb: float = -1.0) -> int:
    q = int(lib().wa_xattn_resident_share(live_clips, T, planes, D, budget_mb))
    if q < 0:
        raise ValueError("bad sizes")
    return q


def xattn_chunk_resident(chunk: int, share: int) -> bool:
    r = int(lib().wa_xattn_chunk_resident(chunk, share))
    if r < 0:
        raise ValueError("bad chunk / share")
    return bool(r)


def xattn_plan(T: int) -> tuple[int, int]:
    s, c = ctypes.c_int(), ctypes.c_int()
    check(lib().wa_xattn_plan(T, ctypes.byref(s), ctypes.byref(c)))
    return s.value, c.value


def xattn_plan_splits(T: int, rows: int, free_cus: int) -> tuple[int, int]:
    s, c = ctypes.c_int(), ctypes.c_int()
    check(lib().wa_xattn_plan_splits(T, rows, free_cus, ctypes.byref(s), ctypes.byref(c)))
    return s.value, c.value


def xattn_kv_check(q, k, v, Tq: int, precision: int = wq4.PREC_F16X2):
    torch = _torch()
    B, H, T, _ = k.shape
    out = torch.empty((B * Tq, 64 * H), device=k.device, dtype=torch.float32)
    dev = k.device.index if k.device.index is not None else 0
    ptr = lambda t: ctypes.c_void_p(t.contiguous().data_ptr())
    check(lib().wa_xattn_kv_check(dev, ptr(q), ptr(k), ptr(v), B, Tq, T, H, precision, ptr(out)))
    return out


def _dev(t) -> int:
    return t.device.index if t.device.index is not None else 0


def _ptr(t):
    return ctypes.c_void_p(t.data_ptr())


def encoder_attention_check(qkv, T: int, H: int, precision: int = wq4.PREC_F16X2):
    torch = _torch()
    qkv = qkv.contiguous()
    B = qkv.shape[0] // T
    out = torch.empty((B * T, 64 * H), device=qkv.device, dtype=torch.float32)
    check(lib().wa_encoder_attention_check(_dev(qkv), _ptr(qkv), B, T, H, precision, _ptr(out)))
    return out


def self_attention_check(qkv, cache_k, cache_v, Tq: int, H: int, kv_len: int, precision: int = wq4.PREC_F16X2):
    torch = _torch()
    B, _, ctx, _ = cache_k.shape
    out = torch.empty((B * Tq, 64 * H), device=qkv.device, dtype=torch.float32)
    check(lib().wa_self_attention_check(_dev(qkv), _ptr(qkv.contiguous()), _ptr(cache_k), _ptr(cache_v), B, Tq, H,
                                        ctx, kv_len, precision, _ptr(out)))
    return out


def logits_argmax_check(hid, emb, step: int, precision: int = wq4.PREC_F16X2, want_logits: bool = True):
    torch = _torch()
    B, D = hid.shape
    V = emb.shape[0]
    tok = torch.empty(B, device=hid.device, dtype=torch.int32)
    lg = torch.empty((B, V), device=hid.device, dtype=torch.float32) if want_logits else None
    check(lib().wa_logits_argmax_check(_dev(hid), _ptr(hid.contiguous()), _ptr(emb.contiguous()), B, D, V, step,
                                       precision, _ptr(tok), _ptr(lg) if lg is not None else None))
    return tok, lg


class GgufReader:

    def __init__(self, path: str):
        h = ctypes.c_void_p(None)
        check(lib().wa_gguf_open(path.encode(), ctypes.byref(h)))
        self._h = h

    @property
    def version(self) -> int:
        return lib().wa_gguf_version(self._h)

    def tensors(self) -> list[dict]:
        out = []
        for i in range(lib().wa_gguf_tensor_count(self._h)):
            name = ctypes.create_string_buffer(512)
            nd, ty = ctypes.c_int(), ctypes.c_int()
            dims = (ctypes.c_uint64 * 8)()
            off, nb = ctypes.c_uint64(), ctypes.c_uint64()
            check(lib().wa_gguf_tensor_info(self._h, i, name, 512, ctypes.byref(nd), dims, ctypes.byref(ty),
                                            ctypes.byref(off), ctypes.byref(nb)))
            out.append({"name": name.value.decode(), "dims": list(dims[: nd.value]), "type": ty.value,
                        "offset": off.value, "nbytes": nb.value})
        return out

    def tensor_data(self, name: str) -> np.ndarray:
        info = next(t for t in self.tensors() if t["name"] == name)
        buf = np.empty(info["nbytes"], np.uint8)
        check(lib().wa_gguf_tensor_data(self._h, name.encode(), buf.ctypes.data_as(ctypes.POINTER(ctypes.c_uint8)),
                                         buf.size))
        return buf

    def close(self):
        if self._h and self._h.value:
            lib().wa_gguf_close(self._h)
            self._h = ctypes.c_void_p(None)

    def __del__(self):
        try:
            self.close()
        except Exception:
            pass


class WhisperModel:

    WEIGHTS = {"q4_0": 0, "f16": 1}

    def __init__(self, variant: str = "large_v3", seed: int = 1234, max_batch: int = 1, device: int = 0,
                 precision: int = wq4.PREC_F16X2, gguf_path: Optional[str] = None, weights: str = "q4_0"):
        h = ctypes.c_void_p(None)
        if gguf_path is None:
            check(lib().wa_model_create_synthetic_ex(device, VARIANTS[variant], seed, max_batch, precision,
                                                     self.WEIGHTS[weights], ctypes.byref(h)))
        else:
            check(lib().wa_model_create_from_gguf(device, gguf_path.encode(), VARIANTS[variant], max_batch,
                                                  precision, ctypes.byref(h)))
        self._h = h
        self.device = device
        self.variant = variant
        self.max_batch = max_batch
        cfg = (ctypes.c_int32 * len(CFG_KEYS))()
        check(lib().wa_model_config(h, cfg))
        self.config = dict(zip(CFG_KEYS, list(cfg)))
        self.weights = {0: "q4_0", 1: "f16"}[lib().wa_model_weight_type(h)]

    @classmethod
    def from_gguf(cls, path: str, variant: str = "large_v3", max_batch: int = 1, device: int = 0,
                  precision: int = wq4.PREC_F16X2) -> "WhisperModel":
        return cls(variant, 0, max_batch, device, precision, gguf_path=path)

    @property
    def wide_range(self) -> bool:
        return lib().wa_model_wide_range(self._h) >= 1

    @property
    def range_tier(self) -> int:
        return lib().wa_model_wide_range(self._h)

    def device_bytes(self) -> int:
        return int(lib().wa_model_device_bytes(self._h))

    def _stream(self):
        return ctypes.c_void_p(_torch().cuda.current_stream(self.device).cuda_stream)

    def transcribe(self, mel, lang_token: Optional[int] = 50259, max_tokens: int = 224, eot_stop: bool = True):
        torch = _torch()
        mel = mel.contiguous()
        assert mel.dtype == torch.float32 and mel.is_cuda
        B = mel.shape[0]
        toks = np.zeros((B, max_tokens), np.int32)
        nt = np.zeros(B, np.int32)
        i32p = ctypes.POINTER(ctypes.c_int32)
        check(lib().wa_transcribe(self._h, ctypes.c_void_p(mel.data_ptr()), B,
                                  -1 if lang_token is None else int(lang_token), max_tokens, 1 if eot_stop else 0,
                                  toks.ctypes.data_as(i32p), nt.ctypes.data_as(i32p), self._stream()))
        return [toks[b, : nt[b]].tolist() for b in range(B)]

    def transcribe_batches(self, mels, lang_token: Optional[int] = 50259, max_tokens: int = 224,
                           eot_stop: bool = True):
        torch = _torch()
        mels = mels.contiguous()
        assert mels.dtype == torch.float32 and mels.is_cuda and mels.dim() == 4
        NB, B = mels.shape[0], mels.shape[1]
        toks = np.zeros((NB, B, max_tokens), np.int32)
        nt = np.zeros((NB, B), np.int32)
        i32p = ctypes.POINTER(ctypes.c_int32)
        check(lib().wa_transcribe_batches(self._h, ctypes.c_void_p(mels.data_ptr()), NB, B,
                                          -1 if lang_token is None else int(lang_token), max_tokens,
                                          1 if eot_stop else 0, toks.ctypes.data_as(i32p), nt.ctypes.data_as(i32p),
                                          self._stream()))
        return [[toks[i, b, : nt[i, b]].tolist() for b in range(B)] for i in range(NB)]

    def pipeline_stats(self) -> dict:
        t = (ctypes.c_float * 4)()
        check(lib().wa_last_pipeline_stats(self._h, t))
        return {"batches": int(t[0]), "overlap_layers": t[1], "masked_ms": t[2], "masked_cus": int(t[3])}

    def pipeline_pairs(self) -> int:
        return int(lib().wa_last_pipeline_pairs(self._h))

    def decode_graph_key(self, group: int = 0) -> int:
        return int(lib().wa_decode_graph_key(self._h, group))

    def transcribe_trace(self, mel, trace_ids: np.ndarray, lang_token: Optional[int] = 50259,
                         max_tokens: int = 224, eot_stop: bool = False):
        torch = _torch()
        mel = mel.contiguous()
        B = mel.shape[0]
        K = trace_ids.shape[-1]
        assert trace_ids.shape == (B, max_tokens + 1, K)
        ids = torch.from_numpy(np.ascontiguousarray(trace_ids, np.int32)).to(mel.device)
        out = torch.full((B, max_tokens + 1, K), float("nan"), device=mel.device, dtype=torch.float32)
        toks = np.zeros((B, max_tokens), np.int32)
        nt = np.zeros(B, np.int32)
        i32p = ctypes.POINTER(ctypes.c_int32)
        check(lib().wa_transcribe_trace(self._h, _ptr(mel), B, -1 if lang_token is None else int(lang_token),
                                        max_tokens, 1 if eot_stop else 0, toks.ctypes.data_as(i32p),
                                        nt.ctypes.data_as(i32p), _ptr(ids), K, _ptr(out), self._stream()))
        return [toks[b, : nt[b]].tolist() for b in range(B)], out.cpu().numpy()

    def transcribe_audio(self, audio, lang_token: Optional[int] = 50259, max_tokens: int = 224,
                         eot_stop: bool = True, n_samples: Optional[int] = None):
        mel = log_mel(audio, self.config["n_mels"], n_samples)
        return self.transcribe(mel, lang_token, max_tokens, eot_stop)

    def last_timings(self) -> dict:
        t = (ctypes.c_float * 5)()
        check(lib().wa_last_timings(self._h, t))
        return {"encoder_ms": t[0], "cross_kv_ms": t[1], "prompt_ms": t[2], "decode_ms": t[3], "steps": int(t[4])}

    PROF_NAMES = ("q4_gemm", "encoder_attention", "conv", "layernorm")

    def profile_enable(self, on: bool = True) -> None:
        check(lib().wa_profile_enable(self._h, 1 if on else 0))

    def profile_read(self, reset: bool = True) -> dict:
        buf = (ctypes.c_double * 16)()
        check(lib().wa_profile_read(self._h, buf, 1 if reset else 0))
        return {n: {"launches": int(buf[4 * i]), "ms": buf[4 * i + 1], "gflop": buf[4 * i + 2], "gb": buf[4 * i + 3]}
                for i, n in enumerate(self.PROF_NAMES)}

    def probe_kernels(self, n_clips: int, iters: int = 20) -> dict:
        buf = (ctypes.c_double * 6)()
        check(lib().wa_probe_kernels(self._h, n_clips, iters, buf, len(buf)))
        return {"cross_attention": {"us": buf[0], "bytes": buf[1], "kv_cache": buf[5] != 0.0},
                "decode_fc1": {"us": buf[2], "bytes": buf[3], "flops": buf[4]}}

    def encode(self, mel):
        torch = _torch()
        B = mel.shape[0]
        out = torch.empty((B, self.config["n_audio_ctx"], self.config["n_audio_state"]), device=mel.device,
                          dtype=torch.float32)
        check(lib().wa_encode(self._h, ctypes.c_void_p(mel.contiguous().data_ptr()), B,
                              ctypes.c_void_p(out.data_ptr()), self._stream()))
        return out

    def prompt_logits(self, prompt):
        torch = _torch()
        B, T = prompt.shape
        out = torch.empty((B, self.config["n_vocab"]), device=prompt.device, dtype=torch.float32)
        check(lib().wa_prompt_logits(self._h, ctypes.c_void_p(prompt.contiguous().data_ptr()), B, T,
                                     ctypes.c_void_p(out.data_ptr()), self._stream()))
        return out

    def close(self):
        if self._h and self._h.value:
            lib().wa_model_destroy(self._h)
            self._h = ctypes.c_void_p(None)

    def __del__(self):
        try:
            self.close()
        except Exception:
            pass
```

Before: 1208.

## Generalize paired decode lanes to up to three concurrent batch lanes

Replaces the fixed two-lane pairing of batches with a generic lane array of up to three lanes. Each lane has its own encoder planes and KV caches, so three batches can decode concurrently on separate groups when batch size is at least 17. The decoder graph cache is widened from one alternate entry to a small ring of kept graphs, so switching between lane keys avoids re-instantiating graphs. It costs extra device memory per lane, and widening can add contention between groups.

```diff
diff --git a/include/whisper_amd.h b/include/whisper_amd.h
--- a/include/whisper_amd.h
+++ b/include/whisper_amd.h
@@ -60,6 +60,8 @@
                                  void* stream);
 wq4_status wa_last_pipeline_stats(const wa_model* m, float* out );
 int wa_last_pipeline_pairs(const wa_model* m);
+int wa_last_pipeline_units3(const wa_model* m);
+wq4_status wa_pipeline_unit_sizes(int n_batches, int width, int* sizes, int* n_units);
 
 wq4_status wa_log_mel(int device, const float* audio_dev, int n_clips, int64_t n_samples, int64_t ld_audio,
                       int n_mels, float* mel_dev, void* stream);
diff --git a/whisper-burn_amd/csrc/whisper/wa_api.cpp b/whisper-burn_amd/csrc/whisper/wa_api.cpp
--- a/whisper-burn_amd/csrc/whisper/wa_api.cpp
+++ b/whisper-burn_amd/csrc/whisper/wa_api.cpp
@@ -204,7 +204,7 @@
   const int B = n_clips, D = c.n_text_state, T = c.n_audio_ctx, H = c.n_text_head;
   DecLayer& L = m->dec[0];
   DecGroup g = m->groups[0];
-  const _Float16* enc = m->enc_planes;
+  const _Float16* enc = m->lanes[0].planes;
   hipEvent_t a, b;
   WA_HIP(hipEventCreate(&a));
   WA_HIP(hipEventCreate(&b));
diff --git a/whisper-burn_amd/csrc/whisper/wa_forward.cpp b/whisper-burn_amd/csrc/whisper/wa_forward.cpp
--- a/whisper-burn_amd/csrc/whisper/wa_forward.cpp
+++ b/whisper-burn_amd/csrc/whisper/wa_forward.cpp
@@ -79,11 +79,12 @@
   m->qkv = f32(renc * 3 * D);
   m->at_d = tiled(renc, D);
   m->at_f = tiled(renc, F);
-  m->enc_planes = d.alloc<_Float16>((size_t)renc * m->ns * D);
+  Lane& lane0 = m->lanes[0];
+  lane0.planes = d.alloc<_Float16>((size_t)renc * m->ns * D);
   m->bytes += (size_t)renc * m->ns * D * 2;
-  for (auto& L : m->dec) {
-    L.cache_k = f32((int64_t)B * c.n_text_ctx * Dt);
-    L.cache_v = f32((int64_t)B * c.n_text_ctx * Dt);
+  for (size_t li = 0; li < m->dec.size(); ++li) {
+    lane0.cache_k.push_back(f32((int64_t)B * c.n_text_ctx * Dt));
+    lane0.cache_v.push_back(f32((int64_t)B * c.n_text_ctx * Dt));
   }
   if (!emb_tiled_supported(Dt)) return fail(WQ4_EINVAL, "n_text_state must be a multiple of 128");
   const size_t erows = (size_t)emb_tiled_rows(c.n_vocab);
@@ -138,12 +139,12 @@
     WA_HIP(hipStreamCreateWithFlags(&g.st, hipStreamNonBlocking));
   }
   m->range_flag = d.alloc<int>(1);
-  for (void* p : {(void*)m->h1, (void*)m->x, (void*)m->qkv, (void*)m->at_d, (void*)m->at_f, (void*)m->enc_planes,
+  for (void* p : {(void*)m->h1, (void*)m->x, (void*)m->qkv, (void*)m->at_d, (void*)m->at_f, (void*)lane0.planes,
                   (void*)m->range_flag})
     if (!p) return fail(WQ4_ENOMEM, "activation allocation failed");
   WA_HIP(hipMemset(m->range_flag, 0, sizeof(int)));
-  for (auto& L : m->dec)
-    if (!L.cache_k || !L.cache_v) return fail(WQ4_ENOMEM, "KV cache allocation failed");
+  for (size_t li = 0; li < m->dec.size(); ++li)
+    if (!lane0.cache_k[li] || !lane0.cache_v[li]) return fail(WQ4_ENOMEM, "KV cache allocation failed");
   WA_HIP(hipMemset(m->at_d, 0, wq4_atiled_bytes(renc, D, m->prec)));
   WA_HIP(hipMemset(m->at_f, 0, wq4_atiled_bytes(renc, F, m->prec)));
   return WQ4_OK;
@@ -236,12 +237,9 @@
 wq4_status cross_kv_forward(wa_model* m, int B, hipStream_t st, bool caches, int lane) {
   const Config& c = m->cfg;
   const int64_t rows = (int64_t)B * c.n_audio_ctx;
-  if (lane == 1) {
-    WA_HIP(launch_enc_planes(m->enc_f32, rows, c.n_audio_state, m->ns, m->enc_planes2, st));
-    return WQ4_OK;
-  }
+  WA_HIP(launch_enc_planes(m->enc_f32, rows, c.n_audio_state, m->ns, m->lanes[lane].planes, st));
+  if (lane > 0) return WQ4_OK;
   m->kv_batch = B;
-  WA_HIP(launch_enc_planes(m->enc_f32, rows, c.n_audio_state, m->ns, m->enc_planes, st));
   m->kv_n = caches && B <= m->kv_small ? B : 0;
   if (m->kv_n > 0 && !m->kv_alloc_ok) {
     const size_t n = (size_t)m->kv_clips * c.n_audio_ctx * c.n_text_state;
@@ -286,7 +284,8 @@
   const int B = g.nb;
   const int64_t rows = (int64_t)B * Tq;
   const size_t self_ofs = (size_t)g.b0 * H * c.n_text_ctx * 64;
-  const _Float16* enc = (g.lane ? m->enc_planes2 : m->enc_planes) + (size_t)g.b0 * T * m->ns * c.n_audio_state;
+  const Lane& lane = m->lanes[g.lane];
+  const _Float16* enc = lane.planes + (size_t)g.b0 * T * m->ns * c.n_audio_state;
   const bool fold = lnfold_on(m, Tq, state, rows);
   float* const a32 = m->f32_attn() ? g.hid : nullptr;
   auto ln_gemm = [&](const wq4_tensor* w, const float* bias, const float* wg, const float* b2, const float* lw,
@@ -322,9 +321,8 @@
   for (int li = 0; li < nl; ++li) {
     DecLayer& L = m->dec[li];
     WA_TRY(ln_gemm(L.qkv, L.qkv_b, L.qkv_wg, L.qkv_b2, L.ln1_w, L.ln1_b, g.qkvd, nullptr, 0u));
-    WA_HIP(launch_decoder_self_attention(g.qkvd, (g.lane ? L.cache_k2 : L.cache_k) + self_ofs,
-                                         (g.lane ? L.cache_v2 : L.cache_v) + self_ofs, B, Tq, H, c.n_text_ctx, state,
-                                         kv0, g.atd_dec, m->ns, st, a32));
+    WA_HIP(launch_decoder_self_attention(g.qkvd, lane.cache_k[li] + self_ofs, lane.cache_v[li] + self_ofs, B, Tq, H,
+                                         c.n_text_ctx, state, kv0, g.atd_dec, m->ns, st, a32));
     WA_TRY(resid_gemm(L.out, L.out_b, g.atd_dec, a32, L.ln2_w));
     WA_TRY(ln_gemm(L.cq, L.cq_b, L.cq_wg, L.cq_b2, L.ln2_w, L.ln2_b, g.qd, nullptr, 0u));
     if (m->group_kv(g)) {
@@ -406,12 +404,25 @@
       ((((((((int64_t)g.lane * 512 + g.b0) * 512 + g.nb) * 2 + (eot_stop ? 1 : 0)) * 2 + (m->trace_out ? 1 : 0)) * 2 +
          (m->group_kv(g) ? 1 : 0)) * 4 + m->range_tier) * 16 + g.xplan.splits) * (kXattnResDen + 1) + g.xres.q;
   if (g.graph && g.graph_key == key) return WQ4_OK;
-  std::swap(g.graph, g.graph_alt);
-  std::swap(g.graph_key, g.graph_alt_key);
-  if (g.graph && g.graph_key == key) return WQ4_OK;
+  for (DecGroup::KeptGraph& k : g.kept)
+    if (k.exec && k.key == key) {
+      std::swap(g.graph, k.exec);
+      std::swap(g.graph_key, k.key);
+      return WQ4_OK;
+    }
   if (g.graph) {
-    (void)hipGraphExecDestroy(g.graph);
+    DecGroup::KeptGraph* slot = nullptr;
+    for (DecGroup::KeptGraph& k : g.kept)
+      if (!k.exec && !slot) slot = &k;
+    if (!slot) {
+      slot = &g.kept[g.kept_next];
+      g.kept_next = (g.kept_next + 1) % kKeptGraphs;
+      (void)hipGraphExecDestroy(slot->exec);
+    }
+    slot->exec = g.graph;
+    slot->key = g.graph_key;
     g.graph = nullptr;
+    g.graph_key = -1;
   }
   WA_WQ4(wq4_prepare_stream(m->device, g.st));
   hipGraph_t gr;
@@ -468,32 +479,31 @@
   return WQ4_OK;
 }
 
-bool ensure_pair_lane(wa_model* m) {
-  if (m->enc_planes2) return true;
+int ensure_lanes(wa_model* m, int want) {
+  want = std::min(want, kMaxLanes);
   const Config& c = m->cfg;
   const size_t np = (size_t)m->bmax * c.n_audio_ctx * m->ns * c.n_audio_state;
   const size_t nc = (size_t)m->bmax * c.n_text_ctx * c.n_text_state;
-  _Float16* planes = m->dev.alloc<_Float16>(np);
-  bool ok = planes != nullptr;
-  for (DecLayer& L : m->dec) {
-    if (!ok) break;
-    L.cache_k2 = m->dev.alloc<float>(nc);
-    L.cache_v2 = m->dev.alloc<float>(nc);
-    ok = L.cache_k2 && L.cache_v2;
-  }
-  if (!ok) {
-    (void)hipGetLastError();
-    m->dev.release(planes);
-    for (DecLayer& L : m->dec) {
-      m->dev.release(L.cache_k2);
-      m->dev.release(L.cache_v2);
-      L.cache_k2 = L.cache_v2 = nullptr;
-    }
-    return false;
-  }
-  m->enc_planes2 = planes;
-  m->bytes += np * 2 + nc * 8 * m->dec.size();
-  return true;
+  while (m->n_lanes < want) {
+    Lane lane;
+    lane.planes = m->dev.alloc<_Float16>(np);
+    bool ok = lane.planes != nullptr;
+    for (size_t li = 0; ok && li < m->dec.size(); ++li) {
+      lane.cache_k.push_back(m->dev.alloc<float>(nc));
+      lane.cache_v.push_back(m->dev.alloc<float>(nc));
+      ok = lane.cache_k.back() && lane.cache_v.back();
+    }
+    if (!ok) {
+      (void)hipGetLastError();
+      m->dev.release(lane.planes);
+      for (float* p : lane.cache_k) m->dev.release(p);
+      for (float* p : lane.cache_v) m->dev.release(p);
+      break;
+    }
+    m->lanes[m->n_lanes++] = std::move(lane);
+    m->bytes += np * 2 + nc * 8 * m->dec.size();
+  }
+  return std::min(m->n_lanes, want);
 }
 
 int decode_groups(int B) {
diff --git a/whisper-burn_amd/csrc/whisper/wa_model.hpp b/whisper-burn_amd/csrc/whisper/wa_model.hpp
--- a/whisper-burn_amd/csrc/whisper/wa_model.hpp
+++ b/whisper-burn_amd/csrc/whisper/wa_model.hpp
@@ -78,13 +78,18 @@
         *fc1_b2 = nullptr;
   uint8_t *ck_raw = nullptr, *cv_raw = nullptr;
   uint32_t* cv_p = nullptr;
-  float *cache_k, *cache_v;
-  float *cache_k2 = nullptr, *cache_v2 = nullptr;
   wq4_tensor *ck = nullptr, *cv = nullptr;
   float *xk = nullptr, *xv = nullptr;
 };
 
+constexpr int kMaxLanes = 3;
+struct Lane {
+  _Float16* planes = nullptr;
+  std::vector<float*> cache_k, cache_v;
+};
+
 constexpr int kMaxGroups = 4;
+constexpr int kKeptGraphs = 4;
 struct DecGroup {
   hipStream_t st = nullptr;
   int b0 = 0, nb = 0;
@@ -109,8 +114,12 @@
   int* host_ndone = nullptr;
   hipGraphExec_t graph = nullptr;
   int64_t graph_key = -1;
-  hipGraphExec_t graph_alt = nullptr;
-  int64_t graph_alt_key = -1;
+  struct KeptGraph {
+    hipGraphExec_t exec = nullptr;
+    int64_t key = -1;
+  };
+  KeptGraph kept[kKeptGraphs];
+  int kept_next = 0;
 };
 
 }
@@ -130,8 +139,8 @@
   std::vector<wa::DecLayer> dec;
   float *h1, *x, *qkv;
   _Float16 *at_d, *at_f;
-  _Float16* enc_planes = nullptr;
-  _Float16* enc_planes2 = nullptr;
+  wa::Lane lanes[wa::kMaxLanes];
+  int n_lanes = 1;
   const float* enc_f32 = nullptr;
   std::vector<wa::DecGroup> groups;
   int wtype = 0;
@@ -147,7 +156,7 @@
   int overlap_k = -1;
   int overlap_b = 0, overlap_eot = -1;
   float pipe[4] = {0, 0, 0, 0};
-  int pipe_pairs = 0;
+  int pipe_pairs = 0, pipe_units3 = 0;
   int* range_flag = nullptr;
   int range_tier = 0;
   bool fold_allowed() const { return range_tier < 1; }
@@ -187,7 +196,8 @@
     resolve_profile();
     for (auto& g : groups) {
       if (g.graph) (void)hipGraphExecDestroy(g.graph);
-      if (g.graph_alt) (void)hipGraphExecDestroy(g.graph_alt);
+      for (auto& k : g.kept)
+        if (k.exec) (void)hipGraphExecDestroy(k.exec);
       if (g.st) (void)hipStreamDestroy(g.st);
       if (g.host_ndone) (void)hipHostFree(g.host_ndone);
     }
@@ -223,7 +233,7 @@
 wq4_status encoder_post(wa_model* m, int B, hipStream_t st, float* enc_out_f32);
 wq4_status encoder_forward(wa_model* m, const float* mel, int B, hipStream_t st, float* enc_out_f32);
 wq4_status cross_kv_forward(wa_model* m, int B, hipStream_t st, bool caches, int lane = 0);
-bool ensure_pair_lane(wa_model* m);
+int ensure_lanes(wa_model* m, int want);
 wq4_status decoder_forward(wa_model* m, DecGroup& g, const int* tokens, int Tq, const DecodeState* state, int pos0,
                            int kv0, hipStream_t st);
 wq4_status prompt_group(wa_model* m, DecGroup& g, int lang_token, hipStream_t st);
diff --git a/whisper-burn_amd/csrc/whisper/wa_transcribe.cpp b/whisper-burn_amd/csrc/whisper/wa_transcribe.cpp
--- a/whisper-burn_amd/csrc/whisper/wa_transcribe.cpp
+++ b/whisper-burn_amd/csrc/whisper/wa_transcribe.cpp
@@ -25,6 +25,7 @@
 };
 
 constexpr int kPairMinClips = 16, kPairMaxClips = 32;
+constexpr int kTripleMinClips = 17;
 
 bool pair_enabled() {
   static const bool enabled = [] {
@@ -34,23 +35,41 @@
   return enabled;
 }
 
-int unit_groups(int B, bool pair) { return pair ? 2 : decode_groups(B); }
-
-wq4_status run_decode(wa_model* m, int B, bool pair, int masked_cus, int lang_token, int max_tokens, int eot_stop,
+int lanes_cap() {
+  static const int cap = [] {
+    const char* e = getenv("WA_LANES");
+    return e ? std::max(1, std::min(kMaxLanes, atoi(e))) : kMaxLanes;
+  }();
+  return cap;
+}
+
+std::vector<int> unit_sizes(int NB, int width) {
+  std::vector<int> sizes;
+  for (int rem = NB; rem > 0; rem -= sizes.back()) {
+    int n = std::min(width, rem);
+    if (rem - n == 1 && n > 2) --n;
+    sizes.push_back(n);
+  }
+  return sizes;
+}
+
+int unit_groups(int B, int n) { return n > 1 ? n : decode_groups(B); }
+
+wq4_status run_decode(wa_model* m, int B, int n, int masked_cus, int lang_token, int max_tokens, int eot_stop,
                       hipEvent_t ready, const hipEvent_t* gprompt, const hipEvent_t* gdone, int* gsteps) {
-  const int G = unit_groups(B, pair);
-  const XattnResidency xres = xattn_residency(pair ? 2 * B : B, m->cfg.n_audio_ctx, m->ns, m->cfg.n_audio_state);
+  const int G = unit_groups(B, n);
+  const XattnResidency xres = xattn_residency(n * B, m->cfg.n_audio_ctx, m->ns, m->cfg.n_audio_state);
   if (m->dev_cus <= 0) WA_HIP(hipDeviceGetAttribute(&m->dev_cus, hipDeviceAttributeMultiprocessorCount, m->device));
-  const int rows = pair ? B : (B + G - 1) / G;
+  const int rows = n > 1 ? B : (B + G - 1) / G;
   const int free_cus = std::max(1, m->dev_cus - masked_cus - (G > 1 ? kXattnPeerCUs : 0));
   const XattnPlan xplan = xattn_plan(m->cfg.n_audio_ctx, rows, free_cus);
   for (int i = 0; i < G; ++i) {
     DecGroup& g = m->groups[i];
     g.xres = xres;
     g.xplan = xplan;
-    g.lane = pair ? i : 0;
-    g.b0 = pair ? 0 : (int)((int64_t)B * i / G);
-    g.nb = pair ? B : (int)((int64_t)B * (i + 1) / G) - g.b0;
+    g.lane = n > 1 ? i : 0;
+    g.b0 = n > 1 ? 0 : (int)((int64_t)B * i / G);
+    g.nb = n > 1 ? B : (int)((int64_t)B * (i + 1) / G) - g.b0;
     WA_HIP(hipStreamWaitEvent(g.st, ready, 0));
     WA_TRY(prompt_group(m, g, lang_token, g.st));
     WA_HIP(hipEventRecord(gprompt[i], g.st));
@@ -96,9 +115,9 @@
   return WQ4_OK;
 }
 
-wq4_status collect_batch(wa_model* m, int B, bool pair, const hipEvent_t* gdone, hipStream_t st, int32_t* tok,
+wq4_status collect_batch(wa_model* m, int B, int n, const hipEvent_t* gdone, hipStream_t st, int32_t* tok,
                          int32_t* nt, int* flag, size_t lane_stride) {
-  const int G = unit_groups(B, pair);
+  const int G = unit_groups(B, n);
   for (int i = 0; i < G; ++i) WA_HIP(hipStreamWaitEvent(st, gdone[i], 0));
   for (int i = 0; i < G; ++i) {
     const DecGroup& g = m->groups[i];
@@ -107,7 +126,7 @@
                           hipMemcpyDeviceToHost, st));
     WA_HIP(hipMemcpyAsync(nt + ofs + g.b0, g.ntok, (size_t)g.nb * 4, hipMemcpyDeviceToHost, st));
   }
-  for (int i = 0; i < (pair ? 2 : 1); ++i)
+  for (int i = 0; i < n; ++i)
     WA_HIP(hipMemcpyAsync(flag + i * lane_stride, m->range_flag, sizeof(int), hipMemcpyDeviceToHost, st));
   return WQ4_OK;
 }
@@ -142,11 +161,11 @@
   WA_TRY(cross_kv_forward(m, B, st, true));
   WA_HIP(hipEventRecord(e_ready, st));
   int gsteps[kMaxGroups] = {};
-  WA_TRY(run_decode(m, B, false, 0, lang_token, max_tokens, eot_stop, e_ready, gprompt, gdone, gsteps));
+  WA_TRY(run_decode(m, B, 1, 0, lang_token, max_tokens, eot_stop, e_ready, gprompt, gdone, gsteps));
   const int steps = *std::max_element(gsteps, gsteps + G);
   std::vector<int32_t> tok((size_t)B * kMaxTokens), nt(B);
   int flag = 0;
-  WA_TRY(collect_batch(m, B, false, gdone, st, tok.data(), nt.data(), &flag, 0));
+  WA_TRY(collect_batch(m, B, 1, gdone, st, tok.data(), nt.data(), &flag, 0));
   WA_HIP(hipEventRecord(e_end, st));
   WA_HIP(hipStreamSynchronize(st));
   *overflow = flag != 0;
@@ -189,8 +208,13 @@
   hipStream_t st = m->own_stream, es = m->enc_stream;
   const int L = (int)m->enc.size();
   const size_t mel_stride = (size_t)B * m->cfg.n_mels * 2 * m->cfg.n_audio_ctx;
-  const bool pairing = pair_enabled() && NB >= 2 && B >= kPairMinClips && B <= kPairMaxClips && B > m->kv_small &&
-                       decode_groups(B) == 2 && ensure_pair_lane(m);
+  int width = 1;
+  if (pair_enabled() && B >= kPairMinClips && B <= kPairMaxClips && B > m->kv_small && decode_groups(B) == 2)
+    width = std::min(lanes_cap(), B >= kTripleMinClips ? kMaxLanes : 2);
+  std::vector<int> sizes = unit_sizes(NB, width);
+  const int widest = *std::max_element(sizes.begin(), sizes.end());
+  const int lanes = ensure_lanes(m, widest);
+  if (lanes < widest) sizes = unit_sizes(NB, lanes);
   int32_t* host = nullptr;
   const size_t per = (size_t)B * kMaxTokens + B + 1;
   WA_HIP(hipHostMalloc(reinterpret_cast<void**>(&host), (size_t)NB * per * 4, 0));
@@ -214,16 +238,15 @@
     hipEvent_t ready, mstart, mend, pstart, gprompt[kMaxGroups], gdone[kMaxGroups];
     int k = 0, gsteps[kMaxGroups] = {};
   };
-  std::vector<Unit> ut;
-  for (int i = 0; i < NB; i += ut.back().n) {
-    ut.emplace_back();
-    ut.back().first = i;
-    ut.back().n = pairing && NB - i >= 2 ? 2 : 1;
-  }
+  std::vector<Unit> ut(sizes.size());
   const int NU = (int)ut.size();
+  for (int i = 0, first = 0; i < NU; first += sizes[i++]) {
+    ut[i].first = first;
+    ut[i].n = sizes[i];
+  }
   for (Unit& u : ut) {
     for (hipEvent_t* e : {&u.ready, &u.mstart, &u.mend, &u.pstart}) WA_HIP(ev.make(e));
-    for (int i = 0; i < unit_groups(B, u.n == 2); ++i) {
+    for (int i = 0; i < unit_groups(B, u.n); ++i) {
       WA_HIP(ev.make(&u.gprompt[i]));
       WA_HIP(ev.make(&u.gdone[i]));
     }
@@ -256,10 +279,9 @@
   int32_t steps_all = 0;
   for (int i = 0; i < NU; ++i) {
     Unit& u = ut[i];
-    const bool pair = u.n == 2;
     if (i >= 1) {
       Unit& p = ut[i - 1];
-      const int PG = unit_groups(B, p.n == 2);
+      const int PG = unit_groups(B, p.n);
       for (int g = 0; g < PG; ++g) WA_HIP(hipEventSynchronize(p.gdone[g]));
       WA_HIP(hipEventSynchronize(p.mend));
       float td = 0.0f, tm = 0.0f;
@@ -285,10 +307,10 @@
       WA_TRY(encoder_layers(m, B, 0, u.k, es));
       WA_HIP(hipEventRecord(u.mend, es));
     }
-    WA_TRY(run_decode(m, B, pair, i + 1 < NU ? m->enc_cus : 0, lang_token, max_tokens, eot_stop, u.ready, u.gprompt,
+    WA_TRY(run_decode(m, B, u.n, i + 1 < NU ? m->enc_cus : 0, lang_token, max_tokens, eot_stop, u.ready, u.gprompt,
                       u.gdone, u.gsteps));
     int32_t* hb = host + (size_t)u.first * per;
-    WA_TRY(collect_batch(m, B, pair, u.gdone, st, hb, hb + (size_t)B * kMaxTokens, hb + (size_t)B * kMaxTokens + B,
+    WA_TRY(collect_batch(m, B, u.n, u.gdone, st, hb, hb + (size_t)B * kMaxTokens, hb + (size_t)B * kMaxTokens + B,
                          per));
     if (i + 1 < NU) {
       WA_HIP(hipStreamWaitEvent(st, u.mend, 0));
@@ -304,9 +326,12 @@
                 n_tokens_out + (size_t)i * B);
     flags[i] = hb[(size_t)B * kMaxTokens + B];
   }
+  int pairs = 0, units3 = 0;
   for (int i = 0; i < NU; ++i) {
     Unit& u = ut[i];
-    const int UG = unit_groups(B, u.n == 2);
+    const int UG = unit_groups(B, u.n);
+    pairs += u.n == 2;
+    units3 += u.n == 3;
     float t = 0.0f, tp = 0.0f, td = 0.0f;
     if (i == 0) {
       WA_HIP(hipEventElapsedTime(&t, e_enc0, u.ready));
@@ -327,7 +352,10 @@
     }
     t_prompt += tp;
     t_decode += td - tp;
-    steps_all += u.n == 2 ? u.gsteps[0] + u.gsteps[1] : *std::max_element(u.gsteps, u.gsteps + UG);
+    if (u.n > 1)
+      for (int g = 0; g < u.n; ++g) steps_all += u.gsteps[g];
+    else
+      steps_all += *std::max_element(u.gsteps, u.gsteps + UG);
   }
   m->timings[0] = (float)(t_exposed / NB);
   m->timings[1] = 0.0f;
@@ -338,7 +366,8 @@
   m->pipe[1] = NU > 1 ? (float)(k_sum / (NU - 1)) : 0.0f;
   m->pipe[2] = NU > 1 ? (float)(t_masked / (NU - 1)) : 0.0f;
   m->pipe[3] = (float)m->enc_cus;
-  m->pipe_pairs = pairing ? NB / 2 : 0;
+  m->pipe_pairs = pairs;
+  m->pipe_units3 = units3;
   return WQ4_OK;
 }
 
@@ -395,6 +424,17 @@
 
 int wa_last_pipeline_pairs(const wa_model* m) { return m ? m->pipe_pairs : 0; }
 
+int wa_last_pipeline_units3(const wa_model* m) { return m ? m->pipe_units3 : 0; }
+
+wq4_status wa_pipeline_unit_sizes(int n_batches, int width, int* sizes, int* n_units) {
+  if (!sizes || !n_units) return fail(WQ4_EINVAL, "null argument");
+  if (n_batches < 1 || width < 1 || width > kMaxLanes) return fail(WQ4_EINVAL, "n_batches >= 1, width in [1, 3]");
+  const std::vector<int> s = unit_sizes(n_batches, width);
+  std::copy(s.begin(), s.end(), sizes);
+  *n_units = (int)s.size();
+  return WQ4_OK;
+}
+
 wq4_status wa_transcribe_trace(wa_model* m, const float* mel_dev, int n_clips, int lang_token, int max_tokens,
                                int eot_stop, int32_t* tokens_out, int32_t* n_tokens_out, const int32_t* trace_ids_dev,
                                int trace_k, float* trace_out_dev, void* stream) {
@@ -409,11 +449,13 @@
   m->trace_out = nullptr;
   m->trace_s1 = m->trace_k = 0;
   for (DecGroup& g : m->groups) {
-    for (hipGraphExec_t* x : {&g.graph, &g.graph_alt}) {
-      if (*x) (void)hipGraphExecDestroy(*x);
-      *x = nullptr;
-    }
-    g.graph_key = g.graph_alt_key = -1;
+    if (g.graph) (void)hipGraphExecDestroy(g.graph);
+    g.graph = nullptr;
+    g.graph_key = -1;
+    for (DecGroup::KeptGraph& k : g.kept) {
+      if (k.exec) (void)hipGraphExecDestroy(k.exec);
+      k = DecGroup::KeptGraph{};
+    }
   }
   return s;
 }
diff --git a/whisper-burn_amd/whisper_amd/__init__.py b/whisper-burn_amd/whisper_amd/__init__.py
--- a/whisper-burn_amd/whisper_amd/__init__.py
+++ b/whisper-burn_amd/whisper_amd/__init__.py
@@ -39,6 +39,10 @@
         L.wa_last_pipeline_stats.argtypes = [vp, f32p]
         L.wa_last_pipeline_pairs.argtypes = [vp]
         L.wa_last_pipeline_pairs.restype = c_int
+        L.wa_last_pipeline_units3.argtypes = [vp]
+        L.wa_last_pipeline_units3.restype = c_int
+        L.wa_pipeline_unit_sizes.argtypes = [c_int, c_int, ctypes.POINTER(c_int), ctypes.POINTER(c_int)]
+        L.wa_pipeline_unit_sizes.restype = c_int
         L.wa_encode.argtypes = [vp, vp, c_int, vp, vp]
         L.wa_prompt_logits.argtypes = [vp, vp, c_int, c_int, vp, vp]
         L.wa_synth_uniform.argtypes = [ctypes.c_uint64, ctypes.c_char_p, c_i64, ctypes.c_float, ctypes.c_float, f32p]
@@ -184,6 +188,12 @@
     return s.value, c.value
 
 
+def pipeline_unit_sizes(n_batches: int, width: int) -> list[int]:
+    sizes, n = (ctypes.c_int * max(1, n_batches))(), ctypes.c_int()
+    check(lib().wa_pipeline_unit_sizes(n_batches, width, sizes, ctypes.byref(n)))
+    return [int(sizes[i]) for i in range(n.value)]
+
+
 def xattn_kv_check(q, k, v, Tq: int, precision: int = wq4.PREC_F16X2):
     torch = _torch()
     B, H, T, _ = k.shape
@@ -346,10 +356,14 @@
     def pipeline_stats(self) -> dict:
         t = (ctypes.c_float * 4)()
         check(lib().wa_last_pipeline_stats(self._h, t))
-        return {"batches": int(t[0]), "overlap_layers": t[1], "masked_ms": t[2], "masked_cus": int(t[3])}
+        return {"batches": int(t[0]), "overlap_layers": t[1], "masked_ms": t[2], "masked_cus": int(t[3]),
+                "pairs": self.pipeline_pairs(), "units3": self.pipeline_units3()}
 
     def pipeline_pairs(self) -> int:
         return int(lib().wa_last_pipeline_pairs(self._h))
+
+    def pipeline_units3(self) -> int:
+        return int(lib().wa_last_pipeline_units3(self._h))
 
     def decode_graph_key(self, group: int = 0) -> int:
         return int(lib().wa_decode_graph_key(self._h, group))
```

Measured after the change: 1323, median of 6. 1.1x the previous value.
